# atonderski/future-object-detection

Measured on AMD Instinct MI355X. Metric: frame-sequences/sec fwd+bwd, T=6 900x1600, higher is better.
Workload: dtype bf16; 1 GPU; spatiotemporal ConditionalDETR (ResNet-50, 6 enc + 6 dec layers, 128 queries), T=6 frames 900x1600, batch 2/GPU, num_images K=5 (5 past frames live), random-init weights; step = forward (incl. Hungarian set loss, post-proc, AP bookkeeping) + backward + clip + AdamW; global_batch=2, frames=6, num_images=5, parallelism=dp1

## Files before the change

future-object-detection_amd/csrc/api.cpp:

```cpp
#include <stdarg.h>
#include <stdio.h>
#include <stdlib.h>
#include <string.h>

#include <mutex>

#include "../../include/fod.h"
#include "knobs.h"

static thread_local char g_err[512] = "";

void fod_set_error(const char* fmt, ...) {
  va_list ap;
  va_start(ap, fmt);
  vsnprintf(g_err, sizeof(g_err), fmt, ap);
  va_end(ap);
}

extern "C" size_t fod_last_error(char* buf, size_t cap) {
  const size_t n = strlen(g_err);
  if (buf && cap) {
    const size_t c = n < cap - 1 ? n : cap - 1;
    memcpy(buf, g_err, c);
    buf[c] = 0;
  }
  return n;
}

extern "C" int fod_abi_version(void) { return FOD_ABI_VERSION; }

extern "C" size_t fod_workspace_bytes(int kind) {
  switch (kind) {
    case FOD_WS_NT_SPLIT: return (size_t)FOD_NT_SPLIT_WS_FLOATS * sizeof(float);
    case FOD_WS_NT_SPLIT_TICKETS: return (size_t)FOD_NT_SPLIT_TICKETS * sizeof(unsigned);
    case FOD_WS_TN_PARTIALS: return FOD_TN_WS_BYTES;
    case FOD_WS_ATTN_SPLIT_PER_TILE: return (size_t)FOD_ATTN_SPLIT_WS_FLOATS_PER_TILE * sizeof(float);
    case FOD_WS_DET: return FOD_DET_WS_BYTES;
    case FOD_WS_TN_MULTI_DET: return FOD_TN_MULTI_DET_WS_BYTES;
    default: return 0;
  }
}

namespace {
struct KnobName {
  const char* name;
  int Knobs::*i;
  double Knobs::*d;
};
const KnobName KNOB_NAMES[] = {
    {"FOD_NT_SMALL", &Knobs::nt_small, nullptr},
    {"FOD_NT_NARROW", &Knobs::nt_narrow, nullptr},
    {"FOD_NT_SPLITK", &Knobs::nt_splitk, nullptr},
    {"FOD_NT_BIG", &Knobs::nt_big, nullptr},
    {"FOD_NT_BIG256", &Knobs::nt_big256, nullptr},
    {"FOD_NT_BIG_ILV", &Knobs::nt_big_ilv, nullptr},
    {"FOD_NT_BIG256_MINK", &Knobs::nt_big256_mink, nullptr},
    {"FOD_NT_BIG_MINK", &Knobs::nt_big_mink, nullptr},
    {"FOD_NT_BIG_MINN", &Knobs::nt_big_minn, nullptr},
    {"FOD_TN_SMALL", &Knobs::tn_small, nullptr},
    {"FOD_TN_BIG", &Knobs::tn_big, nullptr},
    {"FOD_TN_BIG_DENSE", &Knobs::tn_big_dense, nullptr},
    {"FOD_TN_BIG256", &Knobs::tn_big256, nullptr},
    {"FOD_TN_BIG_MIN", nullptr, &Knobs::tn_big_min},
    {"FOD_TN_BIG_SPLITS", &Knobs::tn_big_splits, nullptr},
    {"FOD_TN_WS", &Knobs::tn_ws, nullptr},
    {"FOD_TN_XCD", &Knobs::tn_xcd, nullptr},
    {"FOD_TN_ROWS", &Knobs::tn_rows, nullptr},
    {"FOD_ATTN_LDS", &Knobs::attn_lds, nullptr},
    {"FOD_ATTN_PF", &Knobs::attn_pf, nullptr},
    {"FOD_FP8_STAGE", &Knobs::fp8_stage, nullptr},
    {"FOD_LN_BWD_GROUPS", &Knobs::ln_bwd_groups, nullptr},
    {"FOD_BNK_VERSION", &Knobs::bnk_version, nullptr},
};

bool knob_parse(const KnobName& k, const char* text, Knobs& t) {
  char* end = nullptr;
  if (k.d) {
    const double v = strtod(text, &end);
    if (end == text || *end) return false;
    t.*k.d = v;
    return true;
  }
  if (Knobs{}.*k.i == Knobs::AUTO && !strcmp(text, "auto")) {
    t.*k.i = Knobs::AUTO;
    return true;
  }
  const long v = strtol(text, &end, 10);
  if (end == text || *end || v < 0 || v > 0x7FFFFFFF) return false;
  t.*k.i = (int)v;
  return true;
}

std::mutex g_knob_mutex;
Knobs& knob_table() {
  static Knobs table = [] {
    Knobs t;
    for (const KnobName& k : KNOB_NAMES)
      if (const char* text = getenv(k.name)) knob_parse(k, text, t);
    return t;
  }();
  return table;
}
const KnobName* knob_find(const char* name) {
  for (const KnobName& k : KNOB_NAMES)
    if (name && !strcmp(name, k.name)) return &k;
  fod_set_error("knob: unknown name %s", name ? name : "(null)");
  return nullptr;
}
}

Knobs fod_knobs() {
  std::lock_guard<std::mutex> lock(g_knob_mutex);
  return knob_table();
}

extern "C" int fod_knob_set(const char* name, const char* value) {
  const KnobName* k = knob_find(name);
  if (!k) return FOD_ERR_ARG;
  std::lock_guard<std::mutex> lock(g_knob_mutex);
  Knobs& t = knob_table();
  if (!value) {
    const Knobs def;
    if (k->d) t.*k->d = def.*k->d;
    else t.*k->i = def.*k->i;
  } else if (!knob_parse(*k, value, t)) {
    fod_set_error("knob: %s cannot be '%s'", name, value);
    return FOD_ERR_ARG;
  }
  return FOD_OK;
}

extern "C" int fod_knob_get(const char* name, char* out, size_t out_bytes) {
  const KnobName* k = knob_find(name);
  if (!k) return FOD_ERR_ARG;
  const Knobs t = fod_knobs();
  char text[32];
  int n;
  if (k->d) n = snprintf(text, sizeof(text), "%.17g", t.*k->d);
  else if (t.*k->i == Knobs::AUTO) n = snprintf(text, sizeof(text), "auto");
  else n = snprintf(text, sizeof(text), "%d", t.*k->i);
  if (out && (size_t)n < out_bytes) memcpy(out, text, (size_t)n + 1);
  else {
    fod_set_error("knob: %zu bytes do not hold the value of %s", out_bytes, name);
    return FOD_ERR_ARG;
  }
  return FOD_OK;
}
```

future-object-detection_amd/csrc/elementwise.hip:

```cpp
#include <stdlib.h>

#include "common.h"
#include "det_reduce.h"
#include "knobs.h"

namespace {

constexpr int MAX_BLOCKS = 2048;

FOD_DEVINL long res_row(long m, int div, int mod) {
  unsigned r = (unsigned)m;
  if (div > 0) r /= (unsigned)div;
  if (mod > 0) r %= (unsigned)mod;
  return (long)r;
}

template <int LPR>
FOD_DEVINL float row_sum(float v) {
#pragma unroll
  for (int o = LPR / 2; o > 0; o >>= 1) v += __shfl_xor(v, o);
  return v;
}
template <typename T, int EPL>
struct SliceAlign {
  static constexpr unsigned B = EPL * sizeof(T);
  static constexpr unsigned VALUE = (B & (~B + 1)) > 16 ? 16 : (B & (~B + 1));
};
template <typename T, int EPL>
FOD_DEVINL void ln_load(float* v, const T* p) {
  T t[EPL];
  __builtin_memcpy(t, __builtin_assume_aligned(p, SliceAlign<T, EPL>::VALUE), EPL * sizeof(T));
#pragma unroll
  for (int i = 0; i < EPL; ++i) v[i] = to_f32(t[i]);
}
template <typename T, int EPL>
FOD_DEVINL void ln_store(T* p, const float* v) {
  T t[EPL];
#pragma unroll
  for (int i = 0; i < EPL; ++i) t[i] = from_f32<T>(v[i]);
  __builtin_memcpy(__builtin_assume_aligned(p, SliceAlign<T, EPL>::VALUE), t, EPL * sizeof(T));
}

template <typename T, int D, int LPR>
__global__ __launch_bounds__(256) void ln_fwd_kernel(const T* __restrict__ x, const T* __restrict__ res,
                                                     int rdiv, int rmod, const float* __restrict__ gamma,
                                                     const float* __restrict__ beta, T* __restrict__ y,
                                                     T* __restrict__ sum_out, float* __restrict__ mean,
                                                     float* __restrict__ rstd, int rows, float eps,
                                                     int group_rows) {
  constexpr int EPL = D / LPR, RPW = 64 / LPR;
  const int lane = threadIdx.x & 63;
  const int sub = lane % LPR, rsel = lane / LPR;
  const int c0 = sub * EPL;
  const long rows_per_block = (long)(blockDim.x >> 6) * RPW;
  float ga[EPL], be[EPL];
  __builtin_memcpy(ga, __builtin_assume_aligned(gamma + c0, SliceAlign<float, EPL>::VALUE), EPL * sizeof(float));
  __builtin_memcpy(be, __builtin_assume_aligned(beta + c0, SliceAlign<float, EPL>::VALUE), EPL * sizeof(float));
  for (long base = (long)blockIdx.x * rows_per_block + (threadIdx.x >> 6) * RPW; base < rows;
       base += (long)gridDim.x * rows_per_block) {
    const long row = base + rsel;
    const bool live = row < rows;
    const long r = live ? row : rows - 1;
    if (group_rows > 0) {
      const long goff = (r / group_rows) * D + c0;
      __builtin_memcpy(ga, __builtin_assume_aligned(gamma + goff, SliceAlign<float, EPL>::VALUE), EPL * sizeof(float));
      __builtin_memcpy(be, __builtin_assume_aligned(beta + goff, SliceAlign<float, EPL>::VALUE), EPL * sizeof(float));
    }
    float v[EPL];
    ln_load<T, EPL>(v, x + r * D + c0);
    if (res) {
      float t[EPL];
      ln_load<T, EPL>(t, res + res_row(r, rdiv, rmod) * D + c0);
#pragma unroll
      for (int i = 0; i < EPL; ++i) v[i] += t[i];
    }
    if (sum_out) {
      T st[EPL];
#pragma unroll
      for (int i = 0; i < EPL; ++i) {
        st[i] = from_f32<T>(v[i]);
        v[i] = to_f32(st[i]);
      }
      if (live) __builtin_memcpy(__builtin_assume_aligned(sum_out + r * D + c0, SliceAlign<T, EPL>::VALUE), st, EPL * sizeof(T));
    }
    float s = 0.f;
#pragma unroll
    for (int i = 0; i < EPL; ++i) s += v[i];
    const float mu = row_sum<LPR>(s) * (1.f / D);
    float q = 0.f;
#pragma unroll
    for (int i = 0; i < EPL; ++i) q += (v[i] - mu) * (v[i] - mu);
    const float rs = rsqrtf(row_sum<LPR>(q) * (1.f / D) + eps);
    float o[EPL];
#pragma unroll
    for (int i = 0; i < EPL; ++i) o[i] = (v[i] - mu) * rs * ga[i] + be[i];
    if (live) {
      ln_store<T, EPL>(y + r * D + c0, o);
      if (sub == 0) {
        mean[r] = mu;
        rstd[r] = rs;
      }
    }
  }
}

template <typename T, int D, int LPR, bool DET = false>
__global__ __launch_bounds__(256) void ln_bwd_kernel(const T* __restrict__ dy, const T* __restrict__ xs,
                                                     const float* __restrict__ mean,
                                                     const float* __restrict__ rstd,
                                                     const float* __restrict__ gamma, T* __restrict__ dx,
                                                     float* __restrict__ dgamma, float* __restrict__ dbeta,
                                                     int rows, int group_rows) {
  constexpr int EPL = D / LPR, RPW = 64 / LPR;
  __shared__ float sg[4][D];
  __shared__ float sb[4][D];
  const int lane = threadIdx.x & 63, w = threadIdx.x >> 6;
  const int sub = lane % LPR, rsel = lane / LPR;
  const int c0 = sub * EPL;
  float ga[EPL];
  __builtin_memcpy(ga, __builtin_assume_aligned(gamma + c0, SliceAlign<float, EPL>::VALUE), EPL * sizeof(float));
  float ag[EPL], ab[EPL];
#pragma unroll
  for (int i = 0; i < EPL; ++i) ag[i] = ab[i] = 0.f;
  if (group_rows > 0) {
    const long row = (long)blockIdx.x * 4 + w;
    if (row >= rows) return;
    const long goff = (row / group_rows) * D + c0;
    __builtin_memcpy(ga, __builtin_assume_aligned(gamma + goff, SliceAlign<float, EPL>::VALUE), EPL * sizeof(float));
    const float mu = mean[row], rs = rstd[row];
    float d[EPL], g[EPL], xh[EPL];
    ln_load<T, EPL>(d, dy + row * D + c0);
    ln_load<T, EPL>(xh, xs + row * D + c0);
    float s1 = 0.f, s2 = 0.f;
#pragma unroll
    for (int i = 0; i < EPL; ++i) {
      xh[i] = (xh[i] - mu) * rs;
      g[i] = d[i] * ga[i];
      s1 += g[i];
      s2 += g[i] * xh[i];
    }
    s1 = row_sum<LPR>(s1) * (1.f / D);
    s2 = row_sum<LPR>(s2) * (1.f / D);
    float o[EPL];
#pragma unroll
    for (int i = 0; i < EPL; ++i) o[i] = rs * (g[i] - s1 - xh[i] * s2);
    ln_store<T, EPL>(dx + row * D + c0, o);
#pragma unroll
    for (int i = 0; i < EPL; ++i) {
      if (DET) {
        dgamma[row * (2 * D) + c0 + i] = d[i] * xh[i];
        dgamma[row * (2 * D) + D + c0 + i] = d[i];
      } else {
        atomicAdd(dgamma + goff + i, d[i] * xh[i]);
        atomicAdd(dbeta + goff + i, d[i]);
      }
    }
    return;
  }
  for (long base = (long)blockIdx.x * (4 * RPW) + w * RPW; base < rows; base += (long)gridDim.x * (4 * RPW)) {
    const long row = base + rsel;
    const bool live = row < rows;
    const long r = live ? row : rows - 1;
    const float mu = mean[r], rs = rstd[r];
    float d[EPL], g[EPL], xh[EPL];
    ln_load<T, EPL>(d, dy + r * D + c0);
    ln_load<T, EPL>(xh, xs + r * D + c0);
    float s1 = 0.f, s2 = 0.f;
#pragma unroll
    for (int i = 0; i < EPL; ++i) {
      if (!live) d[i] = 0.f;
      xh[i] = (xh[i] - mu) * rs;
      g[i] = d[i] * ga[i];
      s1 += g[i];
      s2 += g[i] * xh[i];
      ag[i] += d[i] * xh[i];
      ab[i] += d[i];
    }
    s1 = row_sum<LPR>(s1) * (1.f / D);
    s2 = row_sum<LPR>(s2) * (1.f / D);
    float o[EPL];
#pragma unroll
    for (int i = 0; i < EPL; ++i) o[i] = rs * (g[i] - s1 - xh[i] * s2);
    if (live) ln_store<T, EPL>(dx + r * D + c0, o);
  }
#pragma unroll
  for (int i = 0; i < EPL; ++i) {
#pragma unroll
    for (int o = LPR; o < 64; o <<= 1) {
      ag[i] += __shfl_xor(ag[i], o);
      ab[i] += __shfl_xor(ab[i], o);
    }
  }
  if (rsel == 0) {
#pragma unroll
    for (int i = 0; i < EPL; ++i) {
      sg[w][c0 + i] = ag[i];
      sb[w][c0 + i] = ab[i];
    }
  }
  __syncthreads();
  for (int c = threadIdx.x; c < D; c += 256) {
    if (DET) {
      dgamma[(long)blockIdx.x * (2 * D) + c] = sg[0][c] + sg[1][c] + sg[2][c] + sg[3][c];
      dgamma[(long)blockIdx.x * (2 * D) + D + c] = sb[0][c] + sb[1][c] + sb[2][c] + sb[3][c];
    } else {
      atomicAdd(dgamma + c, sg[0][c] + sg[1][c] + sg[2][c] + sg[3][c]);
      atomicAdd(dbeta + c, sb[0][c] + sb[1][c] + sb[2][c] + sb[3][c]);
    }
  }
}

template <typename T>
__global__ void eltwise_vec_kernel(int op, T* __restrict__ out, const T* __restrict__ a, const T* __restrict__ b,
                                   const T* __restrict__ c, unsigned nchunks, int cpr, int bdiv, int bmod,
                                   float alpha) {
  constexpr int VEC = Elem<T>::VEC;
  for (unsigned i = blockIdx.x * blockDim.x + threadIdx.x; i < nchunks; i += gridDim.x * blockDim.x) {
    const unsigned m = i / (unsigned)cpr;
    const unsigned col = (i - m * (unsigned)cpr) * VEC;
    T ta[VEC], tb[VEC], tc[VEC], to[VEC];
    __builtin_memcpy(ta, __builtin_assume_aligned(a + (long)i * VEC, 16), 16);
    if (b) __builtin_memcpy(tb, __builtin_assume_aligned(b + res_row(m, bdiv, bmod) * ((long)cpr * VEC) + col, 16), 16);
    if (op == FOD_EW_ADD3) __builtin_memcpy(tc, __builtin_assume_aligned(c + (long)i * VEC, 16), 16);
#pragma unroll
    for (int e = 0; e < VEC; ++e) {
      const float av = to_f32(ta[e]);
      const float bv = b ? to_f32(tb[e]) : 0.f;
      float r;
      switch (op) {
        case FOD_EW_ADD: r = av + bv; break;
        case FOD_EW_MUL: r = av * bv; break;
        case FOD_EW_RELU_MASK: r = bv > 0.f ? av : 0.f; break;
        case FOD_EW_SCALE: r = alpha * av; break;
        case FOD_EW_ADD3: r = av + bv + to_f32(tc[e]); break;
        case FOD_EW_COPY_B: r = bv; break;
        default: r = fmaxf(av, 0.f); break;
      }
      to[e] = from_f32<T>(r);
    }
    __builtin_memcpy(__builtin_assume_aligned(out + (long)i * VEC, 16), to, 16);
  }
}

template <typename T>
__global__ void eltwise_kernel(int op, T* __restrict__ out, const T* __restrict__ a, const T* __restrict__ b,
                               const T* __restrict__ c, long n, int cols, int bdiv, int bmod, float alpha) {
  for (long i = (long)blockIdx.x * blockDim.x + threadIdx.x; i < n; i += (long)gridDim.x * blockDim.x) {
    const long m = i / cols;
    const int col = (int)(i - m * cols);
    const float av = to_f32(a[i]);
    float bv = 0.f;
    if (b) bv = to_f32(b[res_row(m, bdiv, bmod) * cols + col]);
    float r;
    switch (op) {
      case FOD_EW_ADD: r = av + bv; break;
      case FOD_EW_MUL: r = av * bv; break;
      case FOD_EW_RELU_MASK: r = bv > 0.f ? av : 0.f; break;
      case FOD_EW_SCALE: r = alpha * av; break;
      case FOD_EW_ADD3: r = av + bv + to_f32(c[i]); break;
      case FOD_EW_COPY_B: r = bv; break;
      default: r = fmaxf(av, 0.f); break;
    }
    out[i] = from_f32<T>(r);
  }
}

template <typename TS, typename TD>
__global__ void permute3_kernel(const TS* __restrict__ src, TD* __restrict__ dst, int d0, int d1, int d2, long s0,
                                long s1, long s2, int valid2, const float* __restrict__ scale, int axis) {
  const long n = (long)d0 * d1 * d2;
  for (long i = (long)blockIdx.x * blockDim.x + threadIdx.x; i < n; i += (long)gridDim.x * blockDim.x) {
    const int i2 = (int)(i % d2);
    const long t = i / d2;
    const int i1 = (int)(t % d1);
    const int i0 = (int)(t / d1);
    float v = 0.f;
    if (i2 < valid2) {
      v = to_f32(src[i0 * s0 + i1 * s1 + i2 * s2]);
      if (scale) v *= scale[axis == 0 ? i0 : (axis == 1 ? i1 : i2)];
    }
    dst[i] = from_f32<TD>(v);
  }
}

constexpr int MP_CHUNK = 8192;

__host__ __device__ inline int mp_fast_dim(const fod_permute_job& j) {
  if (j.s2 == 1 || j.d2 == 1) return 2;
  if (j.s1 == 1 && j.d1 > 1) return 1;
  if (j.s0 == 1 && j.d0 > 1) return 0;
  return -1;
}

template <typename TS, typename TD>
FOD_DEVINL void multi_permute_body(const fod_permute_job& j, long chunk, float* tile) {
  const TS* __restrict__ src = reinterpret_cast<const TS*>(j.src);
  TD* __restrict__ dst = reinterpret_cast<TD*>(j.dst);
  const unsigned d0 = j.d0, d1 = j.d1, d2 = j.d2;
  const int fast = mp_fast_dim(j);
  const int tid = threadIdx.x;
  if (fast == 0 || fast == 1) {
    const unsigned df = fast == 1 ? d1 : d0, dg = fast == 1 ? d0 : d1;
    const long sg = fast == 1 ? j.s0 : j.s1;
    const unsigned tiles2 = (d2 + 255) / 256, tilesf = (df + 31) / 32;
    const unsigned c = (unsigned)chunk;
    const unsigned t2 = c % tiles2, rest = c / tiles2;
    const unsigned tf = rest % tilesf, ig = rest / tilesf;
    if (ig >= dg) return;
    const unsigned f0 = tf * 32, c0 = t2 * 256;
    if (df <= 16) {
      TS v[16];
#pragma unroll
      for (unsigned k = 0; k < 16; ++k) {
        const unsigned e = tid + 256 * k;
        const unsigned cc = e / df, ifx = e - cc * df;
        const unsigned i2 = c0 + cc;
        const unsigned i1 = fast == 1 ? ifx : ig;
        const bool ok = k < df && i2 < d2 && i1 < (unsigned)j.valid1 && i2 < (unsigned)j.valid2;
        v[k] = src[ok ? (long)ig * sg + ifx + (long)i2 * j.s2 : 0];
        if (!ok) v[k] = from_f32<TS>(0.f);
      }
#pragma unroll
      for (unsigned k = 0; k < 16; ++k) {
        const unsigned e = tid + 256 * k;
        const unsigned cc = e / df, ifx = e - cc * df;
        if (k < df) tile[ifx * 257 + cc] = to_f32(v[k]);
      }
    } else {
    const unsigned lf = tid & 31, lc = tid >> 5;
    TS v[32];
#pragma unroll
    for (unsigned k = 0; k < 32; ++k) {
      const unsigned cc = lc + 8 * k;
      const unsigned i2 = c0 + cc, ifx = f0 + lf;
      const unsigned i1 = fast == 1 ? ifx : ig;
      const bool ok = ifx < df && i2 < d2 && i1 < (unsigned)j.valid1 && i2 < (unsigned)j.valid2;
      v[k] = src[ok ? (long)ig * sg + ifx + (long)i2 * j.s2 : 0];
      if (!ok) v[k] = from_f32<TS>(0.f);
    }
#pragma unroll
    for (unsigned k = 0; k < 32; ++k) tile[lf * 257 + lc + 8 * k] = to_f32(v[k]);
    }
    __syncthreads();
    if (sizeof(TD) == 2 && c0 + 256 <= d2 && ((j.t0 | j.t1) & 7) == 0 && (reinterpret_cast<uintptr_t>(dst) & 15) == 0) {
      const unsigned l8 = (tid & 31) * 8, rr = tid >> 5;
      for (unsigned r = rr; r < 32; r += 8) {
        const unsigned ifx = f0 + r;
        if (ifx >= df) continue;
        const unsigned i0 = fast == 1 ? ig : ifx, i1 = fast == 1 ? ifx : ig;
        const unsigned i2 = c0 + l8;
        TD o[8];
#pragma unroll
        for (int e = 0; e < 8; ++e) {
          float v = tile[r * 257 + l8 + e];
          if (j.scale) v *= j.scale[j.scale_axis == 0 ? i0 : (j.scale_axis == 1 ? i1 : i2 + e)];
          o[e] = from_f32<TD>(v);
        }
        __builtin_memcpy(__builtin_assume_aligned(dst + (long)i0 * j.t0 + (long)i1 * j.t1 + i2, 16), o, 16);
      }
      return;
// ... 373 lines not shown
}

template <typename T>
__global__ void box_finish_bwd_kernel(const float* __restrict__ dboxes, const float* __restrict__ boxes,
                                      const float* __restrict__ ref, T* __restrict__ dt, float* __restrict__ dref,
                                      int levels, int R, int ref_rows) {
  const int n = ref_rows * 4;
  for (int i = blockIdx.x * blockDim.x + threadIdx.x; i < n; i += gridDim.x * blockDim.x) {
    const int k = i & 3, rr = i >> 2;
    float acc = 0.f;
    for (int l = 0; l < levels; ++l)
      for (int r = rr; r < R; r += ref_rows) {
        const long idx = ((long)l * R + r) * 4 + k;
        const float b = boxes[idx];
        const float g = dboxes[idx] * b * (1.f - b);
        dt[idx] = from_f32<T>(g);
        acc += g;
      }
    if (k < 2) dref[rr * 2 + k] += acc * inv_sigmoid_grad(ref[rr * 2 + k]);
  }
}

inline int grid_for(long n, int per_block = 256) {
  long b = (n + per_block - 1) / per_block;
  if (b > MAX_BLOCKS) b = MAX_BLOCKS;
  if (b < 1) b = 1;
  return (int)b;
}

}

#define FOD_DISPATCH_T(dtype, NAME, ...)                         \
  if ((dtype) == FOD_BF16) { using T = __bf16; __VA_ARGS__; }    \
  else if ((dtype) == FOD_F32) { using T = float; __VA_ARGS__; } \
  else { fod_set_error(NAME ": bad dtype %d", (dtype)); return FOD_ERR_ARG; }

extern "C" int fod_layernorm_fwd(int dtype, const void* x, const void* residual, int res_row_div, int res_row_mod,
                                 const float* gamma, const float* beta, void* y, void* sum_out, float* mean,
                                 float* rstd, int rows, int D, float eps, int group_rows, hipStream_t stream) {
  FOD_REQUIRE(x && gamma && beta && y && mean && rstd && rows > 0, "layernorm_fwd: bad args");
  FOD_REQUIRE(group_rows >= 0 && (group_rows == 0 || rows % group_rows == 0), "layernorm_fwd: %d rows in groups of %d", rows, group_rows);
  FOD_REQUIRE(D % 64 == 0 && D >= 64 && D <= 512, "layernorm_fwd: D=%d must be a multiple of 64, <= 512", D);
  FOD_REQUIRE(((uintptr_t)x % 16) == 0 && ((uintptr_t)y % 16) == 0 && ((uintptr_t)residual % 16) == 0 &&
              ((uintptr_t)sum_out % 16) == 0 && ((uintptr_t)gamma % 16) == 0 && ((uintptr_t)beta % 16) == 0,
              "layernorm_fwd: operands must be 16-byte aligned");
#define LN_FWD(DD)                                                                                            \
  do {                                                                                                        \
    constexpr int LPR = (DD % 128 == 0) ? 16 : 8;                                                             \
    if (rows < 8192) {                                                                                        \
      hipLaunchKernelGGL((ln_fwd_kernel<T, DD, 64>), dim3(grid_for(rows, 4)), dim3(256), 0, stream,           \
                         (const T*)x, (const T*)residual, res_row_div, res_row_mod, gamma, beta, (T*)y,       \
                         (T*)sum_out, mean, rstd, rows, eps, group_rows);                                     \
    } else {                                                                                                  \
      hipLaunchKernelGGL((ln_fwd_kernel<T, DD, LPR>), dim3(grid_for(rows, 4 * (64 / LPR))), dim3(256), 0,     \
                         stream, (const T*)x, (const T*)residual, res_row_div, res_row_mod, gamma, beta,      \
                         (T*)y, (T*)sum_out, mean, rstd, rows, eps, group_rows);                              \
    }                                                                                                         \
  } while (0)
  FOD_DISPATCH_T(dtype, "layernorm_fwd", switch (D / 64) {
    case 1: LN_FWD(64); break; case 2: LN_FWD(128); break; case 3: LN_FWD(192); break; case 4: LN_FWD(256); break;
    case 5: LN_FWD(320); break; case 6: LN_FWD(384); break; case 7: LN_FWD(448); break; default: LN_FWD(512); break; })
#undef LN_FWD
  FOD_LAUNCH_CHECK();
  return FOD_OK;
}

static int ln_bwd_groups() {
  const int n = fod_knobs().ln_bwd_groups;
  return n >= 1 && n <= 16 ? n : 4;
}

extern "C" int fod_layernorm_bwd(int dtype, const void* dy, const void* xsum, const float* mean, const float* rstd,
                                 const float* gamma, void* dx, float* dgamma, float* dbeta, int rows, int D,
                                 int group_rows, hipStream_t stream) {
  FOD_REQUIRE(dy && xsum && mean && rstd && gamma && dx && dgamma && dbeta && rows > 0, "layernorm_bwd: bad args");
  FOD_REQUIRE(group_rows >= 0 && (group_rows == 0 || (rows % group_rows == 0 && rows <= 4096)),
              "layernorm_bwd: %d rows in groups of %d (grouped form: at most 4096 rows)", rows, group_rows);
  FOD_REQUIRE(D % 64 == 0 && D >= 64 && D <= 512, "layernorm_bwd: D=%d must be a multiple of 64, <= 512", D);
  FOD_REQUIRE(((uintptr_t)dy % 16) == 0 && ((uintptr_t)xsum % 16) == 0 && ((uintptr_t)dx % 16) == 0 &&
              ((uintptr_t)gamma % 16) == 0, "layernorm_bwd: operands must be 16-byte aligned");
#define LN_BWD(DD)                                                                                            \
  do {                                                                                                        \
    constexpr int LPR = (DD % 128 == 0) ? 16 : 8;                                                             \
    if (rows < 8192) {                                                                                        \
      int grid = grid_for(rows, 16);                                                                          \
      if (grid > 512) grid = 512;                                                                             \
      if (group_rows > 0) grid = (rows + 3) / 4;                              \
      hipLaunchKernelGGL((ln_bwd_kernel<T, DD, 64>), dim3(grid), dim3(256), 0, stream, (const T*)dy,          \
                         (const T*)xsum, mean, rstd, gamma, (T*)dx, dgamma, dbeta, rows, group_rows);         \
    } else {                                                                                                  \
      int grid = grid_for(rows, 4 * (64 / LPR) * ln_bwd_groups());      \
      if (grid > 512) grid = 512;                                                                             \
      hipLaunchKernelGGL((ln_bwd_kernel<T, DD, LPR>), dim3(grid), dim3(256), 0, stream, (const T*)dy,         \
                         (const T*)xsum, mean, rstd, gamma, (T*)dx, dgamma, dbeta, rows, 0);                  \
    }                                                                                                         \
  } while (0)
  FOD_DISPATCH_T(dtype, "layernorm_bwd", switch (D / 64) {
    case 1: LN_BWD(64); break; case 2: LN_BWD(128); break; case 3: LN_BWD(192); break; case 4: LN_BWD(256); break;
    case 5: LN_BWD(320); break; case 6: LN_BWD(384); break; case 7: LN_BWD(448); break; default: LN_BWD(512); break; })
#undef LN_BWD
  FOD_LAUNCH_CHECK();
  return FOD_OK;
}

extern "C" int fod_layernorm_bwd_det(int dtype, const void* dy, const void* xsum, const float* mean, const float* rstd,
                                     const float* gamma, void* dx, float* dgamma, float* dbeta, int rows, int D,
                                     int group_rows, void* ws, size_t ws_bytes, hipStream_t stream) {
  FOD_REQUIRE_SCRATCH("layernorm_bwd_det", ws, ws_bytes, FOD_DET_WS_BYTES);
  FOD_REQUIRE(dy && xsum && mean && rstd && gamma && dx && dgamma && dbeta && rows > 0, "layernorm_bwd_det: bad args");
  FOD_REQUIRE(group_rows >= 0 && (group_rows == 0 || (rows % group_rows == 0 && rows <= 4096)),
              "layernorm_bwd_det: %d rows in groups of %d (grouped form: at most 4096 rows)", rows, group_rows);
  FOD_REQUIRE(D % 64 == 0 && D >= 64 && D <= 512, "layernorm_bwd_det: D=%d must be a multiple of 64, <= 512", D);
  FOD_REQUIRE(((uintptr_t)dy % 16) == 0 && ((uintptr_t)xsum % 16) == 0 && ((uintptr_t)dx % 16) == 0 &&
              ((uintptr_t)gamma % 16) == 0, "layernorm_bwd_det: operands must be 16-byte aligned");
  float* part = reinterpret_cast<float*>(ws);
  int grid = 0;
  const bool few = rows < 8192;
  if (few) {
    grid = grid_for(rows, 16);
    if (grid > 512) grid = 512;
    if (group_rows > 0) grid = (rows + 3) / 4;
  } else {
    FOD_REQUIRE(group_rows == 0, "layernorm_bwd_det: the grouped form takes at most 4096 rows");
  }
#define LN_BWD_DET(DD)                                                                                        \
  do {                                                                                                        \
    constexpr int LPR = (DD % 128 == 0) ? 16 : 8;                                                             \
    if (few) {                                                                                                \
      hipLaunchKernelGGL((ln_bwd_kernel<T, DD, 64, true>), dim3(grid), dim3(256), 0, stream, (const T*)dy,    \
                         (const T*)xsum, mean, rstd, gamma, (T*)dx, part, nullptr, rows, group_rows);         \
    } else {                                                                                                  \
      grid = grid_for(rows, 4 * (64 / LPR) * ln_bwd_groups());                                                \
      if (grid > 512) grid = 512;                                                                             \
      hipLaunchKernelGGL((ln_bwd_kernel<T, DD, LPR, true>), dim3(grid), dim3(256), 0, stream, (const T*)dy,   \
                         (const T*)xsum, mean, rstd, gamma, (T*)dx, part, nullptr, rows, 0);                  \
    }                                                                                                         \
  } while (0)
  FOD_DISPATCH_T(dtype, "layernorm_bwd_det", switch (D / 64) {
    case 1: LN_BWD_DET(64); break; case 2: LN_BWD_DET(128); break; case 3: LN_BWD_DET(192); break;
    case 4: LN_BWD_DET(256); break; case 5: LN_BWD_DET(320); break; case 6: LN_BWD_DET(384); break;
    case 7: LN_BWD_DET(448); break; default: LN_BWD_DET(512); break; })
#undef LN_BWD_DET
  FOD_LAUNCH_CHECK();
  const int nparts = group_rows > 0 ? group_rows : grid;
  const int groups = group_rows > 0 ? rows / group_rows : 1;
  foddet::ReduceParams r{};
  r.part = part; r.part_stride = 2L * D; r.part_batch = (long)nparts * 2 * D; r.part_total = r.part_batch; r.nparts = nparts;
  r.out0 = dgamma; r.n0 = D; r.cols0 = D; r.ld0 = D; r.out0_batch = D;
  r.out1 = dbeta; r.n1 = D; r.out1_batch = D;
  r.accumulate = 1;
  return det_reduce_launch(r, groups, stream);
}

struct ColsumJob {
  const void* g;
  void* out;
};
constexpr int COLSUM_MAX_JOBS = 16;
struct ColsumJobs {
  ColsumJob j[COLSUM_MAX_JOBS];
};
__global__ __launch_bounds__(256) void colsum_groups_multi_kernel(const ColsumJobs jobs, int group_rows, int N) {
  __shared__ __attribute__((aligned(16))) float red[4][256];
  const int tx = threadIdx.x & 63, rl = threadIdx.x >> 6;
  const int grp = blockIdx.x;
  const __bf16* G = reinterpret_cast<const __bf16*>(jobs.j[blockIdx.y].g) + (long)grp * group_rows * N;
  const bool in = 4 * tx < N;
  float a0 = 0.f, a1 = 0.f, a2 = 0.f, a3 = 0.f;
  if (in) {
    int m = rl;
    for (; m + 28 < group_rows; m += 32) {
      bf16x4_t v[8];
#pragma unroll
      for (int k = 0; k < 8; ++k) v[k] = *reinterpret_cast<const bf16x4_t*>(G + (long)(m + 4 * k) * N + 4 * tx);
#pragma unroll
      for (int k = 0; k < 8; ++k) {
        a0 += (float)v[k][0]; a1 += (float)v[k][1]; a2 += (float)v[k][2]; a3 += (float)v[k][3];
      }
    }
    for (; m < group_rows; m += 4) {
      const bf16x4_t v = *reinterpret_cast<const bf16x4_t*>(G + (long)m * N + 4 * tx);
      a0 += (float)v[0]; a1 += (float)v[1]; a2 += (float)v[2]; a3 += (float)v[3];
    }
  }
  *reinterpret_cast<f32x4*>(&red[rl][4 * tx]) = f32x4{a0, a1, a2, a3};
  __syncthreads();
  if (rl == 0 && in) {
    f32x4 t = *reinterpret_cast<const f32x4*>(&red[0][4 * tx]);
    t += *reinterpret_cast<const f32x4*>(&red[1][4 * tx]);
    t += *reinterpret_cast<const f32x4*>(&red[2][4 * tx]);
    t += *reinterpret_cast<const f32x4*>(&red[3][4 * tx]);
    __bf16* o = reinterpret_cast<__bf16*>(jobs.j[blockIdx.y].out) + (long)grp * N + 4 * tx;
    *reinterpret_cast<bf16x4_t*>(o) = bf16x4_t{(__bf16)t[0], (__bf16)t[1], (__bf16)t[2], (__bf16)t[3]};
  }
}

extern "C" int fod_colsum_groups_multi(int dtype, int njobs, const void* const* ptrs, int groups, int group_rows, int N,
                                       hipStream_t stream) {
  FOD_REQUIRE(dtype == FOD_BF16, "colsum_groups_multi: bf16 only (dtype %d)", dtype);
  FOD_REQUIRE(ptrs && njobs > 0 && njobs <= COLSUM_MAX_JOBS, "colsum_groups_multi: 1 .. %d jobs (%d)", COLSUM_MAX_JOBS, njobs);
  FOD_REQUIRE(groups > 0 && groups <= 65535 && group_rows > 0 && N > 0 && N <= 256 && N % 4 == 0,
              "colsum_groups_multi: %d groups of %d rows, N = %d (N <= 256, a multiple of 4)", groups, group_rows, N);
  ColsumJobs jobs{};
  for (int i = 0; i < njobs; ++i) {
    jobs.j[i].g = ptrs[2 * i];
    jobs.j[i].out = const_cast<void*>(ptrs[2 * i + 1]);
    FOD_REQUIRE(jobs.j[i].g && jobs.j[i].out && ((uintptr_t)jobs.j[i].g % 8) == 0 && ((uintptr_t)jobs.j[i].out % 8) == 0,
                "colsum_groups_multi: job %d: null or misaligned operand", i);
  }
  hipLaunchKernelGGL(colsum_groups_multi_kernel, dim3(groups, njobs), dim3(256), 0, stream, jobs, group_rows, N);
  FOD_LAUNCH_CHECK();
  return FOD_OK;
}

extern "C" int fod_eltwise(int op, int dtype, void* out, const void* a, const void* b, const void* c, long rows,
                           int cols, int b_row_div, int b_row_mod, float alpha, hipStream_t stream) {
  FOD_REQUIRE(out && a && rows > 0 && cols > 0 && rows < (1L << 31), "eltwise: bad args");
  FOD_REQUIRE(op >= FOD_EW_ADD && op <= FOD_EW_COPY_B, "eltwise: bad op %d", op);
  FOD_REQUIRE(b || op == FOD_EW_SCALE || op == FOD_EW_RELU, "eltwise: op %d needs b", op);
  FOD_REQUIRE(c || op != FOD_EW_ADD3, "eltwise: ADD3 needs c");
  const long n = rows * cols;
  const int vec = dtype == FOD_BF16 ? 8 : 4;
  auto al = [](const void* q) { return ((uintptr_t)q % 16) == 0; };
  if (cols % vec == 0 && n / vec < (1L << 32) - 1 && al(out) && al(a) && (!b || al(b)) && (!c || al(c))) {
    FOD_DISPATCH_T(dtype, "eltwise",
                   hipLaunchKernelGGL((eltwise_vec_kernel<T>), dim3(grid_for(n / vec)), dim3(256), 0, stream, op,
                                      (T*)out, (const T*)a, (const T*)b, (const T*)c, (unsigned)(n / vec), cols / vec,
                                      b_row_div, b_row_mod, alpha))
    FOD_LAUNCH_CHECK();
    return FOD_OK;
  }
  FOD_DISPATCH_T(dtype, "eltwise",
                 hipLaunchKernelGGL((eltwise_kernel<T>), dim3(grid_for(n)), dim3(256), 0, stream, op, (T*)out,
                                    (const T*)a, (const T*)b, (const T*)c, n, cols, b_row_div, b_row_mod, alpha))
  FOD_LAUNCH_CHECK();
  return FOD_OK;
}

extern "C" int fod_dropout(int dtype, void* out, const void* a, long n, unsigned long long seed,
                           const unsigned long long* seed_dev, float p, hipStream_t stream) {
  const int vec = dtype == FOD_BF16 ? 8 : 4;
  FOD_REQUIRE(out && a && n > 0 && n % vec == 0 && n < (1L << 32), "dropout: bad size %ld", n);
  FOD_REQUIRE(p >= 0.f && p < 1.f, "dropout: p=%f out of [0, 1)", p);
  FOD_REQUIRE(((uintptr_t)out % 16) == 0 && ((uintptr_t)a % 16) == 0, "dropout: operands must be 16-byte aligned");
  const unsigned threshold = (unsigned)((double)p * 4294967296.0);
  const float inv_keep = 1.f / (1.f - p);
  FOD_DISPATCH_T(dtype, "dropout",
                 hipLaunchKernelGGL((dropout_kernel<T>), dim3(grid_for(n / vec)), dim3(256), 0, stream, (T*)out,
                                    (const T*)a, (unsigned)(n / vec), seed, seed_dev, threshold, inv_keep))
  FOD_LAUNCH_CHECK();
  return FOD_OK;
}

extern "C" int fod_permute3_cast(int src_dtype, int dst_dtype, const void* src, void* dst, int d0, int d1, int d2,
                                 long s0, long s1, long s2, int valid2, const float* scale, int scale_axis,
                                 hipStream_t stream) {
  FOD_REQUIRE(src && dst && d0 > 0 && d1 > 0 && d2 > 0, "permute3: bad args");
  const long n = (long)d0 * d1 * d2;
  const dim3 grid(grid_for(n)), block(256);
#define P3(TS, TD) \
  hipLaunchKernelGGL((permute3_kernel<TS, TD>), grid, block, 0, stream, (const TS*)src, (TD*)dst, d0, d1, d2, s0, s1, s2, valid2, scale, scale_axis)
  if (src_dtype == FOD_F32 && dst_dtype == FOD_F32) P3(float, float);
  else if (src_dtype == FOD_F32 && dst_dtype == FOD_BF16) P3(float, __bf16);
  else if (src_dtype == FOD_BF16 && dst_dtype == FOD_F32) P3(__bf16, float);
  else if (src_dtype == FOD_BF16 && dst_dtype == FOD_BF16) P3(__bf16, __bf16);
  else { fod_set_error("permute3: bad dtypes %d %d", src_dtype, dst_dtype); return FOD_ERR_ARG; }
#undef P3
  FOD_LAUNCH_CHECK();
  return FOD_OK;
}

extern "C" int fod_multi_permute3(const fod_permute_job* jobs, const int* blk_job, const int* blk_chunk, int nblocks,
                                  hipStream_t stream) {
  FOD_REQUIRE(jobs && blk_job && blk_chunk && nblocks > 0, "multi_permute3: bad args");
  hipLaunchKernelGGL(multi_permute3_kernel, dim3(nblocks), dim3(256), 0, stream, jobs, blk_job, blk_chunk);
  FOD_LAUNCH_CHECK();
  return FOD_OK;
}

extern "C" int fod_multi_permute_chunk(void) { return MP_CHUNK; }

extern "C" int fod_multi_permute_tiles(int d0, int d1, int d2, long s0, long s1, long s2) {
  fod_permute_job j{};
  j.d0 = d0; j.d1 = d1; j.d2 = d2; j.s0 = s0; j.s1 = s1; j.s2 = s2;
  const int fast = mp_fast_dim(j);
  if (fast == 0 || fast == 1) {
    const long df = fast == 1 ? d1 : d0, dg = fast == 1 ? d0 : d1;
    return (int)(((d2 + 255) / 256) * ((df + 31) / 32) * dg);
  }
  const long n = (long)d0 * d1 * d2;
  if (n >= (1L << 31)) return -1;
  return (int)((n + MP_CHUNK - 1) / MP_CHUNK);
}

extern "C" int fod_nchw_to_nhwc(int dtype, const float* src, void* dst, int F, int C, int H, int W, int Cp,
                                int inner, long stride_outer, long stride_inner, hipStream_t stream) {
  FOD_REQUIRE(src && dst && F > 0 && C > 0 && Cp >= C && inner > 0 && F % inner == 0, "nchw_to_nhwc: bad args");
  const long n = (long)F * H * W;
  const long hw = (long)H * W;
  if (dtype == FOD_BF16 && Cp == 8 && hw % 4 == 0 && stride_outer % 4 == 0 && stride_inner % 4 == 0 &&
      (reinterpret_cast<uintptr_t>(src) & 15) == 0 && (reinterpret_cast<uintptr_t>(dst) & 15) == 0 && F <= 65535) {
    const int bx = (int)std::min<long>((hw / 4 + 255) / 256, 512);
    hipLaunchKernelGGL(nchw_to_nhwc8_kernel, dim3(bx, F), dim3(256), 0, stream, src, (__bf16*)dst, C, hw, inner,
                       stride_outer, stride_inner);
    FOD_LAUNCH_CHECK();
    return FOD_OK;
// ... 132 lines not shown
```

future-object-detection_amd/csrc/knobs.h:

```cpp
#pragma once

struct Knobs {
  static constexpr int AUTO = -1;
  int nt_small = 1;
  int nt_narrow = AUTO;
  int nt_splitk = AUTO;
  int nt_big = 1;
  int nt_big256 = 1;
  int nt_big_ilv = AUTO;
  int nt_big256_mink = 128;
  int nt_big_mink = 1536;
  int nt_big_minn = 256;
  int tn_small = 1;
  int tn_big = 1;
  int tn_big_dense = 0;
  int tn_big256 = 0;
  double tn_big_min = 2.0e9;
  int tn_big_splits = 0;
  int tn_ws = 1;
  int tn_xcd = 1;
  int tn_rows = 0;
  int attn_lds = 8;
  int attn_pf = 1;
  int fp8_stage = 1;
  int ln_bwd_groups = 4;
  int bnk_version = 4;
};

Knobs fod_knobs();
```

future-object-detection_amd/future_od/models/transformer.py:

```python
import math
from typing import List, Optional

import torch
from torch import Tensor, nn

from future_od.native import functional as Fn
from future_od.native import ops
from future_od.switches import SW


def _reset_parameters(parameters):
    for p in parameters:
        if p.dim() > 1:
            nn.init.xavier_uniform_(p)


def _lin(x, m: nn.Linear, relu=False, out_f32=False):
    return Fn.linear(x, m.weight, m.bias, relu=relu, out_f32=out_f32)


class _Proj:
    __slots__ = ("a", "lin", "a_relu")

    def __init__(self, a, lin, a_relu=False):
# ... 198 lines not shown
    for qc, qs, side, layer, image in blocks:
        kc, ks, _v = side.slots(layer, image)
        jobs.append((qc.detach().contiguous(), qs.detach().contiguous(), kc.detach(), ks.detach()))
    D = blocks[0][0].shape[-1]
    return ops.attn_maps(jobs, 1.0 / math.sqrt(2 * D // nhead), query_idx)


@torch.no_grad()
def _head_mean_weights(qc, kc, qs, ks, H):
    B, M, D = qc.shape
    N = kc.shape[1]
    hd = D // H
    q = torch.cat([qc.float().view(B, M, H, hd), qs.float().view(B, M, H, hd)], 3).transpose(1, 2)
    k = torch.cat([kc.float().view(B, N, H, hd), ks.float().view(B, N, H, hd)], 3).transpose(1, 2)
    w = torch.softmax(q @ k.transpose(-1, -2) / math.sqrt(2 * hd), dim=-1)
    return w.mean(1)


class TransformerDecoderLayer(nn.Module):

    def __init__(self, D, Nhead, Dff=2048, dropout=0.1, num_images=1, use_slotstates=False, use_egodeep=False):
        super().__init__()
        self.self_attend = SlotToSlotAttention(D, Nhead, dropout)
        self.norm_sa = nn.LayerNorm(D)
        self.image_attend = nn.ModuleList([SlotToImageAttention(D, Nhead, dropout) for _ in range(num_images)])
        self.norm_ia = nn.ModuleList([nn.LayerNorm(D) for _ in range(num_images)])
        if use_slotstates:
            self.slotstates_attend = SlotToSlotAttention(D, Nhead, dropout)
            self.norm_ssa = nn.LayerNorm(D)
        else:
            self.slotstates_attend = None
        if use_egodeep:
            self.egodeep_attend = EgodeepAttention(D, Nhead, droprate=dropout, Dff=None)
            self.norm_eda = nn.LayerNorm(D)
        else:
            self.egodeep_attend = None
        self.feedforward = nn.Sequential(nn.Linear(D, Dff), nn.ReLU(inplace=True), nn.Dropout(dropout),
                                         nn.Linear(Dff, D))
        self.norm_out = nn.LayerNorm(D)
        self.Nhead, self.D = Nhead, D
        self.droprate = dropout

    def forward(self, x, qpos, query_sine, side, layer, is_first=False, pos_proj=None, slotstates=None, egodeep=None):
        t, p = self.training, self.droprate
        o = self.self_attend(x, qpos, pos_proj["sa"] if pos_proj else None)
        if side.K > 0:
            x, qc_pre = _add_norm(x, o, self.norm_sa, p, t, then=self.image_attend[0].query_content)
        else:
            x, qc_pre = _add_norm(x, o, self.norm_sa, p, t), None
        qs_all = Fn.group_linear(query_sine, [self.image_attend[i].query_sine for i in range(side.K)])
        for i in range(side.K):
            o, x = self.image_attend[i](x, qpos, query_sine, side, layer, i, is_first, qs=qs_all[i],
                                        qpos_proj=pos_proj["ca"][i] if (pos_proj and is_first) else None, keep=True,
                                        qc_pre=qc_pre)
            if i + 1 < side.K:
                x, qc_pre = _add_norm(x, o, self.norm_ia[i], p, t, then=self.image_attend[i + 1].query_content)
            else:
                x, qc_pre = _add_norm(x, o, self.norm_ia[i], p, t), None
        if self.slotstates_attend is not None and slotstates is not None:
            o = self.slotstates_attend.forward_cross(x, qpos, slotstates)
            x = _add_norm(x, o, self.norm_ssa, p, t)
        if self.egodeep_attend is not None and egodeep is not None and egodeep.dim() == 2 and self.egodeep_attend.per_token_masks():
            egodeep = egodeep.unsqueeze(1)
        if self.egodeep_attend is not None and egodeep is not None and egodeep.dim() == 3:
            e = Fn.dropout(self.egodeep_attend.forward_keys(x, qpos, egodeep), p, t)
            x = Fn.layer_norm(x, self.norm_eda.weight, self.norm_eda.bias, residual=e)
        elif self.egodeep_attend is not None and egodeep is not None:
            e = Fn.dropout(self.egodeep_attend.forward_single_key(egodeep), p, t)
            x = Fn.layer_norm(x, self.norm_eda.weight, self.norm_eda.bias, residual=e, res_row_div=x.shape[1])
            if torch.is_grad_enabled():
                x = Fn.ZeroGradAnchor.apply(x, *self.egodeep_attend.dead_parameters())
        fuse = _fused_tail(self.feedforward[3], p, t)
        x, h = Fn.linear_keep(x, self.feedforward[0].weight, self.feedforward[0].bias, relu=True, grad_masked=fuse)
        h = Fn.dropout(h, p, t)
        return _add_norm(x, _Proj(h, self.feedforward[3], a_relu=fuse), self.norm_out, p, t)


class TransformerDecoder(nn.Module):

    def __init__(self, layers, norm=None, return_intermediate=False, D=256):
        super().__init__()
        self.layers = layers
        for module in self.layers[1:]:
            for att in module.image_attend:
                att.query_pos.weight = None
                att.query_pos.bias = None
        self.norm = norm
        self.return_intermediate = return_intermediate
        self.D = D
        self.query_scale = MLP(D, D, D, 2)
        self.ref_point_head = MLP(D, D, 2, 2)
        _reset_parameters(self.parameters())

    def forward(self, x, qpos, mems, mem_poss, first_layer_special=True, slotstates=None, egodeep=None):
        B, M, D = x.shape
        ref, sine0 = Fn.RefPointSineFn.apply(self.ref_point_head(qpos), D)
        K = len(mems)
        big = [Fn.wide_linear(mems[j], [m for layer in self.layers
                                        for m in (layer.image_attend[j].value, layer.image_attend[j].key_content)])
               for j in range(K)]
        ks_all = Fn.wide_linear(mem_poss[0], [layer.image_attend[j].key_pos for layer in self.layers for j in range(K)])
        side = Fn.MemorySide(big, ks_all, len(self.layers), K, D)
        pos_lin = [m for layer in self.layers for m in (layer.self_attend.query_pos, layer.self_attend.key_pos)]
        if first_layer_special:
            pos_lin += [self.layers[0].image_attend[j].query_pos for j in range(K)]
        pos_all = Fn.group_linear(qpos, pos_lin)
        inter = []
        sine_acc, first_scaled = Fn.TableGradAcc(), True
        for lid, layer in enumerate(self.layers):
            special = lid == 0 and first_layer_special
            pos_proj = {"sa": (pos_all[2 * lid], pos_all[2 * lid + 1]),
                        "ca": pos_all[2 * len(self.layers):] if special else None}
            if special:
                q_sine = sine0
            elif Fn.mlp2_mul_fits(x, self.query_scale, sine0):
                q_sine = Fn.mlp2_mul(x.view(B * M, D), self.query_scale, sine0, acc=sine_acc,
                                     hands_on=first_scaled).view(B, M, D)
                first_scaled = False
            else:
                q_sine = Fn.mul(self.query_scale(x).view(B * M, D), sine0, b_row_mod=M).view(B, M, D)
            x = layer(x, qpos, q_sine, side, lid, is_first=special, pos_proj=pos_proj, slotstates=slotstates,
                      egodeep=egodeep)
            if self.return_intermediate:
                inter.append(x)
        if not self.return_intermediate:
            y = Fn.layer_norm(x, self.norm.weight, self.norm.bias) if self.norm is not None else x
            return y.unsqueeze(0), ref
        return Fn.layer_norm(torch.stack(inter), self.norm.weight, self.norm.bias), ref


class PackedMHA(nn.Module):

    def __init__(self, D):
        super().__init__()
        self.in_proj_weight = nn.Parameter(torch.empty(3 * D, D))
        self.in_proj_bias = nn.Parameter(torch.zeros(3 * D))
        self.out_proj = nn.Linear(D, D)
        nn.init.xavier_uniform_(self.in_proj_weight)
        nn.init.constant_(self.out_proj.bias, 0.0)


class EncoderAttention(nn.Module):

    def __init__(self, Dsrc, num_heads, Dff, droprate=0.1):
        super().__init__()
        self.attn = PackedMHA(Dsrc)
        self.norm1 = nn.LayerNorm(Dsrc)
        self.mlp = nn.Sequential(nn.Linear(Dsrc, Dff), nn.ReLU(inplace=True), nn.Dropout(droprate),
                                 nn.Linear(Dff, Dsrc), nn.Dropout(droprate))
        self.norm2 = nn.LayerNorm(Dsrc)
        self.D, self.H = Dsrc, num_heads
        self.droprate = droprate

    def forward(self, src, pos, other=None, attn_mask=None, key_padding_mask=None):
        _no_masks(attn_mask, key_padding_mask)
        D = self.D
        N = pos.shape[-2]
        add_pos = (lambda t: Fn.add(t, pos, b_row_mod=N)) if pos.dim() == 2 else (lambda t: Fn.add(t, pos))
        fused = Fn.in_proj_self(src, pos, self.attn.in_proj_weight, self.attn.in_proj_bias) if other is None else None
        if fused is not None:
            src, q, k, v = fused
        elif other is None:
            q, k, v = Fn.in_proj(add_pos(src), src, self.attn.in_proj_weight, self.attn.in_proj_bias)
        else:
            q, k, v = Fn.in_proj_cross(add_pos(src), add_pos(other), other, self.attn.in_proj_weight,
                                       self.attn.in_proj_bias)
        a = Fn.attention(q, k, v, 1.0 / math.sqrt(D // self.H), drop_p=self.droprate, training=self.training)
        t, p = self.training, self.droprate
        src = _add_norm(src, _Proj(a, self.attn.out_proj), self.norm1, p, t)
        fuse = _fused_tail(self.mlp[3], p, t)
        src, h = Fn.linear_keep(src, self.mlp[0].weight, self.mlp[0].bias, relu=True, grad_masked=fuse)
        h = Fn.dropout(h, p, t)
        return _add_norm(src, _Proj(h, self.mlp[3], a_relu=fuse), self.norm2, p, t)


class TransformerEncoderLayer(nn.Module):

    def __init__(self, D, Nhead, Dff=2048, droprate=0.1, num_previmages=0, use_prevout=False, use_egodeep=False):
        super().__init__()
        self.self_attn = EncoderAttention(D, Nhead, Dff, droprate=droprate)
        self.prevout_attn = EncoderAttention(D, Nhead, Dff, droprate=droprate) if use_prevout else None
        self.previmage_attn = nn.ModuleList(
            [EncoderAttention(D, Nhead, Dff, droprate=droprate) for _ in range(num_previmages)])
        if use_egodeep:
            self.egodeep_attend = EgodeepAttention(D, Nhead, droprate=droprate, Dff=Dff)
            self.norm_eda = nn.LayerNorm(D)
        else:
            self.egodeep_attend = None

    def forward(self, x, pos, egodeep: Optional[Tensor] = None, prevout: Optional[Tensor] = None, memory=None,
                imu_pre: Optional[Tensor] = None, imu_queue=None):
        x = self.self_attn(x, pos)
        if prevout is not None and self.prevout_attn is not None:
            x = self.prevout_attn(x, pos, other=prevout)
        if memory is not None:
            for prev, attn in zip(memory, self.previmage_attn):
                x = attn(x, pos, other=prev)
        if egodeep is not None and self.egodeep_attend is not None and egodeep.dim() == 2 and self.egodeep_attend.per_token_masks():
            egodeep = egodeep.unsqueeze(1)
        if egodeep is not None and self.egodeep_attend is not None and egodeep.dim() == 3:
            e = self.egodeep_attend.forward_keys(x, pos, egodeep)
            e = Fn.dropout(e, self.egodeep_attend.droprate, self.training)
            x = Fn.layer_norm(x, self.norm_eda.weight, self.norm_eda.bias, residual=e)
        elif egodeep is not None and self.egodeep_attend is not None:
            N = x.shape[1]
            e = imu_pre if imu_pre is not None else self.egodeep_attend.forward_single_key(egodeep)
            e = Fn.dropout(e, self.egodeep_attend.droprate, self.training)
            if imu_queue is not None and e is imu_pre:
                x = Fn.layer_norm(x, self.norm_eda.weight, self.norm_eda.bias, residual=e, res_row_div=N,
                                  res_queue=imu_queue[0], res_slot=imu_queue[1])
            else:
                x = Fn.layer_norm(x, self.norm_eda.weight, self.norm_eda.bias, residual=e, res_row_div=N)
            if torch.is_grad_enabled():
                x = Fn.ZeroGradAnchor.apply(x, *self.egodeep_attend.dead_parameters())
        return x


class TransformerEncoder(nn.Module):
    def __init__(self, layers):
        super().__init__()
        self.layers = layers
        _reset_parameters(self.parameters())

    def forward(self, x, pos, egodeep: Optional[Tensor] = None, prevout: Optional[Tensor] = None, memory=None):
        pre = None
        blocks = [getattr(layer, "egodeep_attend", None) for layer in self.layers]
        if (egodeep is not None and egodeep.dim() == 2 and all(b is not None for b in blocks)
                and not any(b.training and b.droprate > 0.0 for b in blocks) and Fn.imu_branch_fits(egodeep, blocks)):
            queue = Fn.ResGradQueue(len(blocks)) if (SW.FOD_RES_GRAD_QUEUE and torch.is_grad_enabled()) else None
            pre = Fn.imu_branch(egodeep, blocks, queue=queue)
        for i, layer in enumerate(self.layers):
            if pre is not None:
                x = layer(x, pos, egodeep, prevout, memory, imu_pre=pre[i],
                          imu_queue=None if queue is None else (queue, i))
            else:
                x = layer(x, pos, egodeep, prevout, memory)
        return x
```

future-object-detection_amd/future_od/native/functional.py:

```python
import torch
from torch.autograd import Function

from . import lib as L
from . import ops
from .arena import ARENA, _ZeroArena, zeros_f32
from .prepared import (CAT, PREP, STACK, _Job, _Prepared, _VEC, _pad_to, _wkey, prep_conv, prep_linear,
                       prep_stem)
from .wgrad import WGRADS, _WgradQueue
from ..switches import SW

GRAD_SYNC = None


set_deterministic = ops.set_deterministic
is_deterministic = ops.is_deterministic


def set_grad_sync(reducer):
    global GRAD_SYNC
    GRAD_SYNC = reducer


class BackboneCut:

    def __init__(self):
        self.pairs = []

    def cut(self, feat):
        leaf = feat.detach().requires_grad_(True)
        self.pairs.append((feat, leaf))
        return leaf

    def finish(self):
        pairs, self.pairs = self.pairs, []
        if pairs:
            torch.autograd.backward([f for f, _ in pairs], [l.grad for _, l in pairs])


BACKBONE_CUT = None


def cast(t, dtype, pad_cols=None):
    cols = t.shape[-1]
    rows = t.numel() // cols
    t = t.contiguous()
    pc = cols if pad_cols is None else pad_cols
    return ops.permute3_cast(t, dtype, (1, rows, pc), (0, cols, 1), valid2=cols).view(*t.shape[:-1], pc)


def _grad_rows(dy, cols, dtype):
    g = dy.contiguous().view(-1, cols)
    return g if g.dtype == dtype else cast(g, dtype)


def _param_grads(weight, bias, g, x, need_w, need_b, shared):
    want_db = bias is not None and need_b
    if shared and need_w and WGRADS.chain(weight, want_db, g, x):
        return None, None
    db = zeros_f32((g.shape[-1],), x.device) if want_db else None
    dw = None
    if need_w:
        dw = zeros_f32((g.shape[-1], x.shape[-1]), x.device)
        WGRADS.tn(WGRADS.site((weight, bias)), g, x, dw, db, owner=weight if shared else None)
    elif want_db:
        ops.colsum_acc(g, db)
    return dw, db


class LinearFn(Function):

    @staticmethod
    def forward(ctx, x, weight, bias, relu, out_f32):
        dtype = x.dtype
        w = prep_linear(weight, dtype, False)
        N = weight.shape[0]
        y = ops.gemm_nt(x, w[:N] if w.shape[0] != N else w, shift=bias, relu=relu, out_f32=out_f32)
        y = y.view(*x.shape[:-1], N)
        ctx.relu, ctx.out_f32 = relu, out_f32
        ctx.weight, ctx.bias = weight, bias
        ctx.has_bias = bias is not None
        ctx.save_for_backward(x, y if relu else None)
        return y

    @staticmethod
    def backward(ctx, dy):
        x, y = ctx.saved_tensors
        weight = ctx.weight
        dtype = x.dtype
        N, K = weight.shape
        v = _VEC[dtype]
        Np = _pad_to(N, v)
        dy = dy.contiguous()
        if dy.dtype != dtype or Np != N:
            g = cast(dy.view(-1, N), dtype, pad_cols=Np)
        else:
            g = dy.view(-1, N)
        if ctx.relu:
            assert Np == N
            g = ops.eltwise(L.EW_RELU_MASK, g, y.view(-1, N))
        dx = None
        if ctx.needs_input_grad[0]:
            dx = ops.gemm_nt(g, prep_linear(weight, dtype, True)).view(x.shape)
        dw, db = _param_grads(weight, ctx.bias, g, x.view(-1, K), ctx.needs_input_grad[1], ctx.needs_input_grad[2], True)
        if Np != N:
            dw, db = (None if dw is None else dw[:N]), (None if db is None else db[:N])
        return dx, dw, db, None, None


def linear(x, weight, bias=None, relu=False, out_f32=False):
    return LinearFn.apply(x.contiguous(), weight, bias, relu, out_f32)


class LinearKeepFn(Function):

    @staticmethod
    def forward(ctx, x, weight, bias, relu, grad_masked=False, precomputed=None):
        dtype = x.dtype
        N = weight.shape[0]
        if precomputed is not None:
            y = precomputed.view(*x.shape[:-1], N)
        else:
            w = prep_linear(weight, dtype, False)
            y = ops.gemm_nt(x, w[:N] if w.shape[0] != N else w, shift=bias, relu=relu).view(*x.shape[:-1], N)
        ctx.relu, ctx.weight, ctx.bias, ctx.has_bias = relu, weight, bias, bias is not None
        ctx.mask_here = relu and not grad_masked
        ctx.save_for_backward(x, y if ctx.mask_here else None)
        return x.view_as(x), y

    @staticmethod
    def backward(ctx, dkeep, dy):
        x, y = ctx.saved_tensors
        weight = ctx.weight
        dtype = x.dtype
        N, K = weight.shape
        assert N % _VEC[dtype] == 0
        g = _grad_rows(dy, N, dtype)
        if ctx.mask_here:
            g = ops.eltwise(L.EW_RELU_MASK, g, y.view(-1, N))
        dx = None
        if ctx.needs_input_grad[0]:
            res = None if dkeep is None else _grad_rows(dkeep, K, dtype)
            dx = ops.gemm_nt(g, prep_linear(weight, dtype, True), residual=res).view(x.shape)
        dw, db = _param_grads(weight, ctx.bias, g, x.view(-1, K), ctx.needs_input_grad[1], ctx.needs_input_grad[2], False)
        return dx, dw, db, None, None, None


def linear_keep(x, weight, bias=None, relu=False, grad_masked=False, precomputed=None):
    if weight.shape[0] % _VEC[x.dtype] != 0 or not SW.FOD_LINEAR_KEEP:
        assert precomputed is None
        return x, linear(x, weight, bias, relu=relu)
    return LinearKeepFn.apply(x.contiguous(), weight, bias, relu, grad_masked, precomputed)


class AddFn(Function):

    @staticmethod
    def forward(ctx, a, b, b_row_div, b_row_mod):
        ctx.cfg = (b_row_div, b_row_mod, b.shape, a.shape)
        return ops.eltwise(L.EW_ADD, a, b, b_row_div=b_row_div, b_row_mod=b_row_mod)

    @staticmethod
    def backward(ctx, g):
        div, mod, bshape, ashape = ctx.cfg
        g = g.contiguous()
        db = None
        if ctx.needs_input_grad[1]:
            cols = ashape[-1]
            rows = g.numel() // cols
            if not div and not mod:
                db = g.view(bshape)
            elif mod and not div:
                db = _sum_periodic(g.view(rows, cols), mod).view(bshape)
            else:
                assert not mod
                out = zeros_f32((rows // div, cols), g.device)
                ops.colsum_acc(g.view(rows, cols), out, group_rows=div)
                db = cast(out, g.dtype).view(bshape)
        return (g.view(ashape) if ctx.needs_input_grad[0] else None), db, None, None


def add(a, b, b_row_div=0, b_row_mod=0):
    return AddFn.apply(a.contiguous(), b.contiguous(), b_row_div, b_row_mod)


class MulFn(Function):

    @staticmethod
    def forward(ctx, a, b, b_row_mod):
        ctx.save_for_backward(a, b)
        ctx.mod = b_row_mod
        return ops.eltwise(L.EW_MUL, a, b, b_row_mod=b_row_mod)

    @staticmethod
    def backward(ctx, g):
        a, b = ctx.saved_tensors
        g = g.contiguous()
        da = ops.eltwise(L.EW_MUL, g, b, b_row_mod=ctx.mod)
        db = ops.eltwise(L.EW_MUL, g, a)
        if ctx.mod:
            db = _sum_periodic(db, ctx.mod).view(b.shape)
        return da, db, None


class TableGradAcc:

    def __init__(self):
        self.buf = None

    def get(self, shape, device):
        if self.buf is None:
            self.buf = zeros_f32(shape, device)
        return self.buf

    def take(self):
        buf, self.buf = self.buf, None
        return buf


class Mlp2MulFn(Function):

    @staticmethod
    def forward(ctx, x, table, w1, b1, w2, b2, acc, hands_on):
        D = x.shape[-1]
        x2 = x.view(-1, D)
        out, h, q = ops.mlp2_mul_fwd(x2, prep_linear(w1, x.dtype, False), b1, prep_linear(w2, x.dtype, False), b2, table)
        ctx.save_for_backward(x2, h, q, table)
        ctx.params, ctx.acc, ctx.hands_on, ctx.x_shape = (w1, b1, w2, b2), acc, hands_on, x.shape
        return out.view(x.shape)

    @staticmethod
    def backward(ctx, g):
        x2, h, q, table = ctx.saved_tensors
        w1, b1, w2, b2 = ctx.params
        D = x2.shape[-1]
        g = _grad_rows(g, D, x2.dtype)
        acc = ctx.acc if ctx.acc is not None else TableGradAcc()
        buf = acc.get(tuple(table.shape), x2.device)
        ds, dh, dx = ops.mlp2_mul_bwd(g, table, q, h, prep_linear(w2, x2.dtype, True), prep_linear(w1, x2.dtype, True), buf)
        dw2, db2 = _param_grads(w2, b2, ds, h, ctx.needs_input_grad[4], ctx.needs_input_grad[5], True)
        dw1, db1 = _param_grads(w1, b1, dh, x2, ctx.needs_input_grad[2], ctx.needs_input_grad[3], True)
        dtable = None
        if ctx.needs_input_grad[1] and (ctx.acc is None or ctx.hands_on):
            dtable = cast(acc.take(), table.dtype).view(table.shape)
        return (dx.view(ctx.x_shape) if ctx.needs_input_grad[0] else None), dtable, dw1, db1, dw2, db2, None, None


def mlp2_mul_fits(x, mlp, table):
    if not SW.FOD_FUSED_MLP2 or x.dtype != torch.bfloat16 or getattr(mlp, "num_layers", 0) != 2:
        return False
    l0, l1 = mlp.layers
    D = x.shape[-1]
    return (D == 256 and tuple(l0.weight.shape) == (D, D) and tuple(l1.weight.shape) == (D, D) and l0.bias is not None
            and l1.bias is not None and table.dtype == x.dtype and table.dim() == 2 and table.shape[1] == D
            and (x.numel() // D) % table.shape[0] == 0)


def mlp2_mul(x, mlp, table, acc=None, hands_on=True):
    l0, l1 = mlp.layers
    return Mlp2MulFn.apply(x.contiguous(), table.contiguous(), l0.weight, l0.bias, l1.weight, l1.bias, acc, hands_on)


def _sum_periodic(g, mod):
    parts = g.view(-1, mod, g.shape[-1])
# ... 260 lines not shown
DROP_SEEDS = _DropSeeds()


def manual_seed(seed):
    torch.manual_seed(seed)
    DROP_SEEDS.count = 0
    if ops.DROP_BASE is not None:
        ops.DROP_BASE.zero_()


class DropoutFn(Function):
    @staticmethod
    def forward(ctx, x, p, seed):
        ctx.p, ctx.seed = p, seed
        return ops.dropout(x, p, seed)

    @staticmethod
    def backward(ctx, g):
        return ops.dropout(g.contiguous(), ctx.p, ctx.seed), None, None


def dropout(x, p, training):
    if not training or p <= 0.0:
        return x
    return DropoutFn.apply(x.contiguous(), float(p), DROP_SEEDS.next())


def _fp8_takes(q1, k1, drop_p):
    mode = SW.FOD_ATTN_FP8
    if mode == "off" or q1.dtype != torch.bfloat16 or drop_p > 0.0:
        return False
    few_queries = q1.shape[1] <= 512 and k1.shape[1] >= 128
    return mode == "all" or not few_queries


class AttentionFn(Function):
    @staticmethod
    def forward(ctx, q1, k1, v, q2, k2, scale, drop_p=0.0, drop_seed=0):
        ctx.drop = (drop_p, drop_seed)
        ctx.scale = scale
        ctx.two = q2 is not None
        ctx.fp8 = _fp8_takes(q1, k1, drop_p)
        if ctx.fp8:
            need_bwd = any(t is not None and t.requires_grad for t in (q1, k1, v, q2, k2))
            o, lse2, deq = ops.attn_fwd_fp8(q1, k1, v, scale, q2, k2, want_backward=need_bwd)
            if need_bwd:
                ctx.save_for_backward(deq[0], deq[1], deq[2], deq[3], deq[4], o, lse2)
            return o
        o, lse2 = ops.attn_fwd(q1, k1, v, scale, q2, k2, drop_p=drop_p, drop_seed=drop_seed)
        ctx.save_for_backward(q1, k1, v, q2, k2, o, lse2)
        return o

    @staticmethod
    def backward(ctx, do):
        q1, k1, v, q2, k2, o, lse2 = ctx.saved_tensors
        slots = {}
        qk = _column_siblings(q1, k1)
        if qk is not None:
            D = q1.shape[-1]
            dqk = torch.empty_strided(qk.shape, qk.stride(), dtype=qk.dtype, device=qk.device)
            slots = dict(dq1_out=dqk[..., :D], dk1_out=dqk[..., D:])
        elif q1.shape == k1.shape == v.shape and q1.is_contiguous() and k1.is_contiguous() and v.is_contiguous():
            buf = torch.empty((3,) + tuple(q1.shape), dtype=q1.dtype, device=q1.device)
            slots = dict(dq1_out=buf[0], dk1_out=buf[1], dv_out=buf[2])
        if ctx.fp8:
            dq1, dk1, dq2, dk2, dv = ops.attn_bwd(q1, k1, v, o, do.contiguous(), lse2, 1.0 / ops.LOG2E, q2, k2,
                                                  dq_scale=ctx.scale * ops.LOG2E, **slots)
            return dq1, dk1, dv, dq2, dk2, None, None, None
        dq1, dk1, dq2, dk2, dv = ops.attn_bwd(q1, k1, v, o, do.contiguous(), lse2, ctx.scale, q2, k2,
                                              drop_p=ctx.drop[0], drop_seed=ctx.drop[1], **slots)
        return dq1, dk1, dv, dq2, dk2, None, None, None


def _strided_ok(t):
    v = _VEC[t.dtype]
    return (t.dim() == 3 and t.stride(-1) == 1 and t.stride(0) % v == 0 and t.stride(1) % v == 0
            and t.data_ptr() % 16 == 0)


def attention(q1, k1, v, scale, q2=None, k2=None, drop_p=0.0, training=False):
    c = lambda t: None if t is None else (t if _strided_ok(t) else t.contiguous())
    drop = (float(drop_p), DROP_SEEDS.next()) if training and drop_p > 0.0 else ()
    return AttentionFn.apply(c(q1), c(k1), c(v), c(q2), c(k2), scale, *drop)


def _column_siblings(a, b):
    D = a.shape[-1]
    if (b is None or a.shape != b.shape or a.stride() != b.stride() or a.stride(-1) != 1 or a.stride(-2) != 2 * D
            or a.untyped_storage().data_ptr() != b.untyped_storage().data_ptr()
            or b.storage_offset() != a.storage_offset() + D):
        return None
    outer = 2 * D
    for n, st in zip(reversed(a.shape[:-1]), reversed(a.stride()[:-1])):
        if st != outer:
            return None
        outer *= n
    return torch.as_strided(a, tuple(a.shape[:-1]) + (2 * D,), a.stride())


class InProjFn(Function):

    @staticmethod
    def forward(ctx, xp, src, w, b):
        return _in_proj_forward(ctx, xp, src, w, b)

    @staticmethod
    def backward(ctx, dq, dk, dv):
        return _in_proj_backward(ctx, dq, dk, dv, ctx.needs_input_grad[0], ctx.needs_input_grad[1])


def _in_proj_forward(ctx, xp, src, w, b):
    D = w.shape[1]
    dtype = xp.dtype
    wqk, wv = prep_linear(w[:2 * D], dtype, False), prep_linear(w[2 * D:], dtype, False)
    qk = ops.gemm_nt(xp, wqk, shift=b[:2 * D]).view(*xp.shape[:-1], 2 * D)
    v = ops.gemm_nt(src, wv, shift=b[2 * D:]).view(src.shape)
    ctx.save_for_backward(xp, src)
    ctx.w, ctx.b = w, b
    return qk[..., :D], qk[..., D:], v


def _in_proj_backward(ctx, dq, dk, dv, need_xp, need_src, chained=False, dkeep=None):
    xp, src = ctx.saved_tensors
    w, b = ctx.w, ctx.b
    D = w.shape[1]
    dtype = xp.dtype
    rows = xp.numel() // D
    dqk = _column_siblings(dq, dk)
    if dqk is None:
        dqk = torch.cat([dq, dk], dim=-1)
    dqk = dqk.reshape(rows, 2 * D)
    dv = dv.contiguous().view(rows, D)
    dxp = dsrc = None
    if need_xp:
        res = None if dkeep is None else _grad_rows(dkeep, D, dtype)
        dxp = ops.gemm_nt(dqk, prep_linear(w[:2 * D], dtype, True), residual=res).view(xp.shape)
    if need_src:
        dsrc = ops.gemm_nt(dv, prep_linear(w[2 * D:], dtype, True), residual=dxp if chained else None).view(src.shape)
    dw = zeros_f32((3 * D, D), xp.device)
    db = zeros_f32((3 * D,), xp.device)
    wq = WGRADS.site((w, b))
    WGRADS.tn(wq, dqk, xp.view(rows, D), dw[:2 * D], db[:2 * D])
    WGRADS.tn(wq, dv, src.view(rows, D), dw[2 * D:], db[2 * D:])
    return dxp, dsrc, dw, db


def in_proj(xp, src, weight, bias):
    return InProjFn.apply(xp.contiguous(), src.contiguous(), weight, bias)


class InProjSelfFn(Function):

    @staticmethod
    def forward(ctx, src, pos, w, b, row_mod):
        xp = ops.eltwise(L.EW_ADD, src, pos, b_row_mod=row_mod)
        return (src.view_as(src),) + _in_proj_forward(ctx, xp, src, w, b)

    @staticmethod
    def backward(ctx, dkeep, dq, dk, dv):
        need = ctx.needs_input_grad[0]
        _, dsrc, dw, db = _in_proj_backward(ctx, dq, dk, dv, need, need, chained=True, dkeep=dkeep)
        return dsrc, None, dw, db, None


def in_proj_self(src, pos, weight, bias):
    if pos.requires_grad or not SW.FOD_LINEAR_KEEP:
        return None
    row_mod = pos.shape[-2] if pos.dim() == 2 else 0
    return InProjSelfFn.apply(src.contiguous(), pos.contiguous(), weight, bias, row_mod)


class InProjCrossFn(Function):

    @staticmethod
    def forward(ctx, xq, xk, xv, w, b):
        D = w.shape[1]
        dtype = xq.dtype
        q = ops.gemm_nt(xq, prep_linear(w[:D], dtype, False), shift=b[:D]).view(xq.shape)
        k = ops.gemm_nt(xk, prep_linear(w[D:2 * D], dtype, False), shift=b[D:2 * D]).view(xk.shape)
        v = ops.gemm_nt(xv, prep_linear(w[2 * D:], dtype, False), shift=b[2 * D:]).view(xv.shape)
        ctx.save_for_backward(xq, xk, xv)
        ctx.w, ctx.b = w, b
        return q, k, v

    @staticmethod
    def backward(ctx, dq, dk, dv):
        xs = ctx.saved_tensors
        w, b = ctx.w, ctx.b
        D = w.shape[1]
        dtype = xs[0].dtype
        dw = zeros_f32((3 * D, D), xs[0].device)
        db = zeros_f32((3 * D,), xs[0].device)
        dxs = []
        wq = WGRADS.site((w, b))
        for i, (x, g) in enumerate(zip(xs, (dq, dk, dv))):
            rows = x.numel() // D
            g = g.contiguous().view(rows, D)
            sl = slice(i * D, (i + 1) * D)
            dxs.append(ops.gemm_nt(g, prep_linear(w[sl], dtype, True)).view(x.shape) if ctx.needs_input_grad[i] else None)
            WGRADS.tn(wq, g, x.view(rows, D), dw[sl], db[sl])
        return dxs[0], dxs[1], dxs[2], dw, db


def in_proj_cross(xq, xk, xv, weight, bias):
    return InProjCrossFn.apply(xq.contiguous(), xk.contiguous(), xv.contiguous(), weight, bias)


class RefPointSineFn(Function):

    @staticmethod
    def forward(ctx, ref_logit, D):
        ref, sine = ops.refpoint_sine_fwd(ref_logit, D)
        ctx.save_for_backward(ref)
        ctx.D, ctx.act_dtype = D, ref_logit.dtype
        return ref, sine

    @staticmethod
    def backward(ctx, dref, dsine):
        (ref,) = ctx.saved_tensors
        if dsine is None:
            dsine = torch.zeros((ref.shape[0], ctx.D), dtype=ctx.act_dtype, device=ref.device)
        return ops.refpoint_sine_bwd(dsine.contiguous(), ref, None if dref is None else dref.contiguous()), None


class BoxFinishFn(Function):

    @staticmethod
    def forward(ctx, t, ref, levels):
        boxes = ops.box_finish_fwd(t, ref, levels)
        ctx.save_for_backward(boxes, ref)
        ctx.act_dtype = t.dtype
        ctx.t_shape = t.shape
        return boxes

    @staticmethod
    def backward(ctx, dboxes):
        boxes, ref = ctx.saved_tensors
        dt_, dref = ops.box_finish_bwd(dboxes.contiguous(), boxes, ref, ctx.act_dtype)
        return dt_.view(ctx.t_shape), dref, None


class ZeroGradAnchor(Function):

    @staticmethod
    def forward(ctx, x, *params):
        ctx.shapes = [(p.shape, p.device) for p in params]
        return x.view_as(x)

    @staticmethod
    def backward(ctx, g):
        return (g,) + tuple(zeros_f32(s, d) for s, d in ctx.shapes)


class CastFn(Function):

    @staticmethod
    def forward(ctx, x, dtype, pad_cols):
        ctx.src_dtype, ctx.cols = x.dtype, x.shape[-1]
        return cast(x, dtype, pad_cols)

    @staticmethod
    def backward(ctx, g):
        g = g.contiguous()
        cols = g.shape[-1]
        rows = g.numel() // cols
        out = ops.permute3_cast(g, ctx.src_dtype, (1, rows, ctx.cols), (0, cols, 1))
        return out.view(*g.shape[:-1], ctx.cols), None, None


def cast_ad(x, dtype, pad_cols=None):
    if x.dtype == dtype and pad_cols in (None, x.shape[-1]):
        return x
    return CastFn.apply(x.contiguous(), dtype, pad_cols)




class WideLinearFn(Function):

    @staticmethod
    def forward(ctx, x, *params):
        P = len(params) // 2
        weights, biases = params[:P], params[P:]
        wcat, bcat, _ = CAT.get(weights, biases, x.dtype)
        y = ops.gemm_nt(x, wcat, shift=bcat).view(*x.shape[:-1], wcat.shape[0])
        ctx.save_for_backward(x)
        ctx.params = params
        return y

    @staticmethod
    def backward(ctx, dy):
        (x,) = ctx.saved_tensors
        P = len(ctx.params) // 2
        weights, biases = ctx.params[:P], ctx.params[P:]
        D_out, D_in = weights[0].shape
        _, _, wcat_t = CAT.get(weights, biases, x.dtype)
        g = dy.contiguous().view(-1, P * D_out)
        dx = None
        if ctx.needs_input_grad[0]:
            dx = ops.gemm_nt(g, wcat_t).view(x.shape)
        dw = zeros_f32((P * D_out, D_in), x.device)
        db = zeros_f32((P * D_out,), x.device)
        WGRADS.tn(WGRADS.site(ctx.params), g, x.view(-1, D_in), dw, db)
        gw = [dw[i * D_out:(i + 1) * D_out] for i in range(P)]
        gb = [db[i * D_out:(i + 1) * D_out] for i in range(P)]
        return (dx,) + tuple(gw) + tuple(gb)


class GroupLinearFn(Function):

    @staticmethod
    def forward(ctx, x, nres, res_mod, *tensors):
        res, params = tensors[:nres], tensors[nres:]
        P = len(params) // 2
        weights, biases = params[:P], params[P:]
        wcat, bcat, _ = CAT.get(weights, biases, x.dtype)
        D = weights[0].shape[0]
        rblock = None
        if nres:
            rblock = _as_segments(res, res[0].numel() // D, D)
            assert rblock is not None, "group_linear(residual=...): the tables must be consecutive blocks (the caller checks)"
        y = ops.group_linear_fwd(x.view(-1, x.shape[-1]), wcat, bcat, P, residual=rblock, res_row_mod=res_mod)
# ... 301 lines not shown
```

future-object-detection_amd/future_od/native/ops.py:

```python
import ctypes as C
import math

import torch

from . import abi, capture
from . import lib as L
from .lib import F32, BF16, AttnShape, ConvGeom, Epilogue
from .. import switches
from ..switches import SW


def call(name, *args, **kw):
    return L.call(name, *args, **kw)

_DT = {torch.float32: F32, torch.bfloat16: BF16}


def dt(t):
    try:
        return _DT[t.dtype]
    except KeyError:
        raise L.FodError(f"unsupported activation dtype {t.dtype}") from None


# ... 848 lines not shown
    if out is None:
        out = torch.empty((B, Q, n, S), dtype=torch.float32, device=q1.device)
    else:
        _chk(out, f"{who}: out", torch.float32)
        if tuple(out.shape) != (B, Q, n, S) or out.device != q1.device:
            raise L.FodError(f"{who}: out {tuple(out.shape)} is not [{B}, {Q}, {n}, {S}] on {q1.device}")
    H = E // 32
    shp = AttnShape(B, H, Tq, S, qb, qt, kb, kt, 0, 0, 0, 0, float(scale), k2b, k2t, 0, 0, 0.0, 0, None, None, None, 0.0)
    parts = 2 if q2 is not None else 1
    call("fod_attn_maps", dt(q1), n, C.addressof(arr), ptr(query_idx), Q, ptr(out), _Addr(shp), stream(),
         work=2.0 * 2 * n * B * H * Q * S * 32 * parts)
    return out


def layernorm_fwd(x, gamma, beta, residual=None, res_row_div=0, res_row_mod=0, want_sum=None, eps=1e-5, group_rows=0):
    _chk(x, "x"); _chk(gamma, "gamma", torch.float32); _chk(beta, "beta", torch.float32)
    D = x.shape[-1]
    rows = x.numel() // D
    if group_rows:
        assert rows % group_rows == 0 and gamma.numel() == (rows // group_rows) * D and beta.numel() == gamma.numel()
    else:
        assert gamma.numel() == D and beta.numel() == D
    if residual is not None:
        _chk(residual, "residual", x.dtype); assert residual.shape[-1] == D
        rr = residual.numel() // D
        need = rows
        if res_row_div:
            need = (rows - 1) // res_row_div + 1
        if res_row_mod:
            need = min(need, res_row_mod)
        assert rr >= need, (x.shape, residual.shape, res_row_div, res_row_mod)
    want_sum = (residual is not None) if want_sum is None else want_sum
    y = torch.empty_like(x)
    s = torch.empty_like(x) if want_sum else None
    mean = torch.empty(rows, dtype=torch.float32, device=x.device)
    rstd = torch.empty(rows, dtype=torch.float32, device=x.device)
    call("fod_layernorm_fwd", dt(x), ptr(x), ptr(residual), res_row_div, res_row_mod, ptr(gamma), ptr(beta),
         ptr(y), ptr(s), ptr(mean), ptr(rstd), rows, D, eps, group_rows, stream())
    return y, (s if want_sum else x), mean, rstd


def linear_add_norm_fwd(a, w, bias, x, gamma, beta, eps=1e-5, then_w=None, then_bias=None):
    _chk(a, "a", torch.bfloat16); _chk(w, "w", torch.bfloat16); _chk(x, "x", torch.bfloat16)
    _chk(gamma, "gamma", torch.float32); _chk(beta, "beta", torch.float32)
    N, K = w.shape
    M = a.numel() // K
    assert a.shape[-1] == K and x.numel() == M * N and gamma.numel() == N and beta.numel() == N, (a.shape, w.shape, x.shape)
    if bias is not None:
        _chk(bias, "bias", torch.float32); assert bias.numel() == N
    y = torch.empty_like(x)
    s = torch.empty_like(x)
    mean = torch.empty(M, dtype=torch.float32, device=x.device)
    rstd = torch.empty(M, dtype=torch.float32, device=x.device)
    out2 = None
    if then_w is not None:
        _chk(then_w, "then_w", torch.bfloat16); assert tuple(then_w.shape) == (N, N)
        if then_bias is not None:
            _chk(then_bias, "then_bias", torch.float32); assert then_bias.numel() == N
        out2 = torch.empty_like(x)
    call("fod_linear_add_norm_fwd", dt(a), ptr(a), K, ptr(w), ptr(bias), ptr(x), ptr(gamma), ptr(beta), ptr(y), ptr(s),
         ptr(mean), ptr(rstd), M, N, K, eps, ptr(then_w), ptr(then_bias), ptr(out2), stream(),
         work=2.0 * M * N * K * (2 if then_w is not None else 1), tag="fod_gemm_nt")
    return (y, s, mean, rstd) if then_w is None else (y, s, mean, rstd, out2)


def linear_add_norm_bwd(dy, xsum, mean, rstd, gamma, w_t, dgamma, dbeta, want_da=True, pre_g=None, pre_w_t=None):
    _chk(xsum, "xsum", torch.bfloat16); _chk(w_t, "w_t", torch.bfloat16)
    K, N = w_t.shape
    M = xsum.numel() // N
    if pre_g is not None:
        _chk(pre_g, "pre_g", torch.bfloat16); _chk(pre_w_t, "pre_w_t", torch.bfloat16)
        assert pre_g.numel() == M * N and tuple(pre_w_t.shape) == (N, N)
    else:
        assert pre_w_t is None and dy is not None
    if dy is not None:
        _chk(dy, "dy", torch.bfloat16); assert dy.numel() == xsum.numel()
    assert mean.numel() == M and rstd.numel() == M and gamma.numel() == N
    _chk(dgamma, "dgamma", torch.float32); _chk(dbeta, "dbeta", torch.float32)
    dsum = torch.empty_like(xsum)
    da = torch.empty((M, K), dtype=xsum.dtype, device=xsum.device) if want_da else None
    call_twin("fod_linear_add_norm_bwd", xsum.device, dt(xsum), ptr(dy), ptr(xsum), ptr(mean), ptr(rstd), ptr(gamma),
              ptr(w_t), ptr(dsum), ptr(da), ptr(dgamma), ptr(dbeta), M, N, K, ptr(pre_g), ptr(pre_w_t),
              work=2.0 * M * N * K * ((1 if want_da else 0) + (1 if pre_g is not None else 0)), tag="fod_gemm_nt")
    return dsum, da


def colsum_groups_multi(jobs, groups, group_rows, N):
    n = len(jobs)
    assert 0 < n <= 16
    arr = (C.c_void_p * (2 * n))()
    for i, (g, out) in enumerate(jobs):
        _chk(g, "g", torch.bfloat16); _chk(out, "out", torch.bfloat16)
        assert g.numel() == groups * group_rows * N and out.numel() == groups * N
        arr[2 * i], arr[2 * i + 1] = g.data_ptr(), out.data_ptr()
    call("fod_colsum_groups_multi", BF16, n, C.addressof(arr), groups, group_rows, N, stream())


def mlp2_mul_fwd(x, w1, b1, w2, b2, table=None):
    _chk(x, "x", torch.bfloat16); _chk(w1, "w1", torch.bfloat16); _chk(w2, "w2", torch.bfloat16)
    D = x.shape[-1]
    M = x.numel() // D
    assert tuple(w1.shape) == (D, D) and tuple(w2.shape) == (D, D), (x.shape, w1.shape, w2.shape)
    for b in (b1, b2):
        if b is not None:
            _chk(b, "bias", torch.float32); assert b.numel() == D
    rows_t = 0
    if table is not None:
        _chk(table, "table", torch.bfloat16); assert table.shape[-1] == D
        rows_t = table.numel() // D
        assert M % rows_t == 0
    h = torch.empty((M, D), dtype=x.dtype, device=x.device)
    q = torch.empty((M, D), dtype=x.dtype, device=x.device) if table is not None else None
    out = torch.empty((M, D), dtype=x.dtype, device=x.device)
    call("fod_mlp2_mul_fwd", dt(x), ptr(x), ptr(w1), ptr(b1), ptr(w2), ptr(b2), ptr(table), rows_t, ptr(h), ptr(q),
         ptr(out), M, D, stream(), work=4.0 * M * D * D, tag="fod_gemm_nt")
    return out, h, q


def mlp2_mul_bwd(dout, table, q, h, w2_t, w1_t, dtable):
    _chk(dout, "dout", torch.bfloat16); _chk(h, "h", torch.bfloat16)
    _chk(w2_t, "w2_t", torch.bfloat16); _chk(w1_t, "w1_t", torch.bfloat16)
    D = dout.shape[-1]
    M = dout.numel() // D
    assert h.numel() == M * D and tuple(w2_t.shape) == (D, D) and tuple(w1_t.shape) == (D, D)
    rows_t = 0
    ds = None
    if table is not None:
        _chk(table, "table", torch.bfloat16); _chk(q, "q", torch.bfloat16); _chk(dtable, "dtable", torch.float32)
        rows_t = table.numel() // D
        assert q.numel() == M * D and dtable.numel() == rows_t * D and M % rows_t == 0
        ds = torch.empty((M, D), dtype=dout.dtype, device=dout.device)
    dh = torch.empty((M, D), dtype=dout.dtype, device=dout.device)
    dx = torch.empty((M, D), dtype=dout.dtype, device=dout.device)
    call_twin("fod_mlp2_mul_bwd", dout.device, dt(dout), ptr(dout), ptr(table), rows_t, ptr(q), ptr(h), ptr(w2_t),
              ptr(w1_t), ptr(ds), ptr(dh), ptr(dx), ptr(dtable), M, D, work=4.0 * M * D * D, tag="fod_gemm_nt")
    return (ds if table is not None else dout), dh, dx


def layernorm_bwd(dy, xsum, mean, rstd, gamma, dgamma, dbeta, group_rows=0):
    _chk(dy, "dy"); _chk(xsum, "xsum", dy.dtype)
    D = dy.shape[-1]
    rows = dy.numel() // D
    assert xsum.numel() == dy.numel() and mean.numel() == rows and rstd.numel() == rows
    groups = rows // group_rows if group_rows else 1
    assert not group_rows or (rows % group_rows == 0 and rows <= 4096)
    for t in (gamma, dgamma, dbeta):
        _chk(t, "gamma/dgamma/dbeta", torch.float32); assert t.numel() == groups * D
    dx = torch.empty_like(dy)
    call_twin("fod_layernorm_bwd", dy.device, dt(dy), ptr(dy), ptr(xsum), ptr(mean), ptr(rstd), ptr(gamma), ptr(dx),
              ptr(dgamma), ptr(dbeta), rows, D, group_rows)
    return dx


def eltwise(op, a, b=None, c=None, b_row_div=0, b_row_mod=0, alpha=1.0, out=None):
    _chk(a, "a")
    cols = a.shape[-1]
    rows = a.numel() // cols
    if b is not None:
        _chk(b, "b", a.dtype); assert b.shape[-1] == cols
        need = rows
        if b_row_div:
            need = (rows - 1) // b_row_div + 1
        if b_row_mod:
            need = min(need, b_row_mod)
        assert b.numel() // cols >= need, (a.shape, b.shape, b_row_div, b_row_mod)
    if c is not None:
        _chk(c, "c", a.dtype); assert c.numel() == a.numel()
    out = torch.empty_like(a) if out is None else out
    call("fod_eltwise", op, dt(a), ptr(out), ptr(a), ptr(b), ptr(c), rows, cols, b_row_div, b_row_mod,
         float(alpha), stream())
    return out


def add(a, b, **kw):
    return eltwise(L.EW_ADD, a, b, **kw)


DROP_BASE = None


def dropout(a, p, seed):
    _chk(a, "a")
    out = torch.empty_like(a)
    call("fod_dropout", dt(a), ptr(out), ptr(a), a.numel(), seed & 0xFFFFFFFFFFFFFFFF, ptr(DROP_BASE), float(p), stream())
    return out


def posenc_table(h, w, c, dtype, device, temperature=10000.0):
    out = torch.empty((h * w, c), dtype=dtype, device=device)
    call("fod_posenc_table", _DT[dtype], ptr(out), h, w, c, temperature, stream())
    return out


def posenc_temporal(b, l, c, dtype, device, offsets=None, extra=0.0, temperature=10000.0):
    out = torch.empty((b, l, c), dtype=dtype, device=device)
    if offsets is not None:
        _chk(offsets, "offsets", torch.float32); assert offsets.shape == (b, l)
    call("fod_posenc_temporal", _DT[dtype], ptr(out), ptr(offsets), b, l, c, extra, temperature, stream())
    return out


def refpoint_sine_fwd(ref_logit, D):
    _chk(ref_logit, "ref_logit")
    R = ref_logit.numel() // 2
    ref = torch.empty((R, 2), dtype=torch.float32, device=ref_logit.device)
    sine = torch.empty((R, D), dtype=ref_logit.dtype, device=ref_logit.device)
    call("fod_refpoint_sine_fwd", dt(ref_logit), ptr(ref_logit), ptr(ref), ptr(sine), R, D, stream())
    return ref, sine


def refpoint_sine_bwd(dsine, ref, dref_extra):
    _chk(dsine, "dsine"); _chk(ref, "ref", torch.float32)
    R, D = dsine.shape
    assert ref.shape == (R, 2)
    if dref_extra is not None:
        _chk(dref_extra, "dref_extra", torch.float32); assert dref_extra.shape == (R, 2)
    out = torch.empty((R, 2), dtype=dsine.dtype, device=dsine.device)
    call("fod_refpoint_sine_bwd", dt(dsine), ptr(dsine), ptr(ref), ptr(dref_extra), ptr(out), R, D, stream())
    return out


def box_finish_fwd(t, ref, levels):
    _chk(t, "t"); _chk(ref, "ref", torch.float32)
    ref_rows = ref.shape[0]
    assert t.numel() % (levels * 4) == 0
    R = t.numel() // (levels * 4)
    assert R % ref_rows == 0 and ref.shape == (ref_rows, 2)
    boxes = torch.empty((levels, R, 4), dtype=torch.float32, device=t.device)
    call("fod_box_finish_fwd", dt(t), ptr(t), ptr(ref), ptr(boxes), levels, R, ref_rows, stream())
    return boxes


def box_finish_bwd(dboxes, boxes, ref, act_dtype):
    _chk(dboxes, "dboxes", torch.float32); _chk(boxes, "boxes", torch.float32)
    levels, R, _ = boxes.shape
    ref_rows = ref.shape[0]
    assert dboxes.shape == boxes.shape and ref.shape == (ref_rows, 2) and R % ref_rows == 0
    dt_ = torch.empty((levels, R, 4), dtype=act_dtype, device=boxes.device)
    dref = torch.zeros((ref_rows, 2), dtype=torch.float32, device=boxes.device)
    call("fod_box_finish_bwd", _DT[act_dtype], ptr(dboxes), ptr(boxes), ptr(ref), ptr(dt_), ptr(dref),
         levels, R, ref_rows, stream())
    return dt_, dref


def match_cost(logits, boxes, tgt_labels, tgt_boxes, tgt_offset, ld_n, w_class, w_bbox, w_giou,
               alpha=0.25, gamma=2.0):
    _chk(logits, "logits", torch.float32); _chk(boxes, "boxes", torch.float32)
    Lv, B, M, Cc = logits.shape
    assert boxes.shape == (Lv, B, M, 4) and tgt_offset.dtype == torch.int32 and tgt_offset.numel() == B + 1
    cost = torch.zeros((Lv, B, M, ld_n), dtype=torch.float32, device=logits.device)
    call("fod_match_cost", ptr(logits), ptr(boxes), ptr(tgt_labels), ptr(tgt_boxes), ptr(tgt_offset),
         ptr(cost), Lv, B, M, Cc, ld_n, w_class, w_bbox, w_giou, alpha, gamma, stream())
    return cost


def lap_solve_batch_host(cost_cpu, n_cols, threads=8):
    assert cost_cpu.device.type == "cpu" and cost_cpu.dtype == torch.float32 and cost_cpu.is_contiguous()
    P, M, ld = cost_cpu.shape
    nc = torch.tensor(n_cols, dtype=torch.int32)
    assert nc.numel() == P
    out = torch.empty((P, M), dtype=torch.int32)
    call("fod_lap_solve_batch_host", cost_cpu.data_ptr(), P, M, ld, nc.data_ptr(), out.data_ptr(), threads)
    return out


def _num_boxes_args(num_boxes):
    if isinstance(num_boxes, torch.Tensor):
        _chk(num_boxes, "num_boxes", torch.float32); assert num_boxes.numel() == 1
        return 1.0, num_boxes
    return float(num_boxes), None


def set_loss_fwd(logits, boxes, match, tgt_labels, tgt_boxes, tgt_offset, num_boxes, alpha):
    Lv, B, M, Cc = logits.shape
    _chk(match, "match", torch.int32); assert match.shape == (Lv, B, M)
    out = torch.empty((Lv, 5), dtype=torch.float32, device=logits.device)
    nb, nb_dev = _num_boxes_args(num_boxes)
    call("fod_set_loss_fwd", ptr(logits), ptr(boxes), ptr(match), ptr(tgt_labels), ptr(tgt_boxes),
         ptr(tgt_offset), ptr(out), Lv, B, M, Cc, nb, ptr(nb_dev), alpha, stream())
    return out


def set_loss_bwd(logits, boxes, match, tgt_labels, tgt_boxes, g, num_boxes, alpha):
    Lv, B, M, Cc = logits.shape
    _chk(g, "g", torch.float32); assert g.shape == (Lv, 3)
    dlogits, dboxes = torch.empty_like(logits), torch.empty_like(boxes)
    nb, nb_dev = _num_boxes_args(num_boxes)
    call("fod_set_loss_bwd", ptr(logits), ptr(boxes), ptr(match), ptr(tgt_labels), ptr(tgt_boxes), ptr(g),
         ptr(dlogits), ptr(dboxes), Lv, B, M, Cc, nb, ptr(nb_dev), alpha, stream())
    return dlogits, dboxes


def pack_targets_dev(anno_boxes, anno_classes, anno_active, H, W):
    _chk(anno_boxes, "anno_boxes", torch.float32); _chk(anno_classes, "anno_classes", torch.int64)
    _chk(anno_active, "anno_active", torch.int64)
    B, N = anno_classes.shape
    assert anno_boxes.shape == (B, N, 4) and anno_active.shape == (B, N)
    dev = anno_boxes.device
    labels = torch.empty((B * N,), dtype=torch.int64, device=dev)
    boxes = torch.empty((B * N, 4), dtype=torch.float32, device=dev)
    offset = torch.empty((B + 1,), dtype=torch.int32, device=dev)
    count = torch.empty((1,), dtype=torch.float32, device=dev)
    call("fod_pack_targets", ptr(anno_boxes), ptr(anno_classes), ptr(anno_active), B, N, 1 / W, 1 / H, ptr(labels),
         ptr(boxes), ptr(offset), ptr(count), stream())
    return {"labels": labels, "boxes": boxes, "offset": offset, "count": count, "ld": N, "device": True}

# ... 100 lines not shown
```

include/fod.h:

```cpp
#ifndef FOD_H_
#define FOD_H_

#include <stddef.h>
#include <stdint.h>

#ifdef __cplusplus
extern "C" {
#endif

typedef struct ihipStream_t* fod_stream_t;

enum { FOD_F32 = 0, FOD_BF16 = 1 };
enum { FOD_OK = 0, FOD_ERR_ARG = 1, FOD_ERR_LAUNCH = 2, FOD_ERR_RUNTIME = 3 };

size_t fod_last_error(char* buf, size_t cap);
int fod_abi_version(void);
#define FOD_ABI_VERSION 15

int fod_knob_set(const char* name, const char* value);
int fod_knob_get(const char* name, char* out, size_t out_bytes);

enum { FOD_ROUTE_NT_SMALL = 0,
       FOD_ROUTE_NT_128 = 1,
       FOD_ROUTE_NT_BIG = 2 };
typedef struct fod_nt_route {
  int kernel;
  int tile_n;
  int stages;
  int interleave;
  int ksplit;
  int wants_split_ws;
} fod_nt_route;
enum { FOD_ROUTE_TN_SMALL = 0,
       FOD_ROUTE_TN_128 = 1,
       FOD_ROUTE_TN_BIG = 2 };
typedef struct fod_tn_route {
  int kernel;
  int bi, bj;
  int nsplit;
  int m_per_split;
  int xcd_order;
  int uses_partials_ws;
} fod_tn_route;

typedef struct fod_epilogue {
  const float* scale;
  const float* shift;
  const void* residual;
  long ld_residual;
  int residual_row_mod;
  const void* relu_mask;
  long ld_mask;
  int relu;
  int out_f32;
  void* split_ws;
  void* split_tickets;
} fod_epilogue;
#define FOD_NT_SPLIT_WS_FLOATS (64 * 8 * 4096)
#define FOD_NT_SPLIT_TICKETS 64
#define FOD_TN_WS_BYTES ((size_t)64 << 20)
enum { FOD_WS_NT_SPLIT = 0, FOD_WS_NT_SPLIT_TICKETS = 1, FOD_WS_TN_PARTIALS = 2, FOD_WS_ATTN_SPLIT_PER_TILE = 3,
       FOD_WS_DET = 4, FOD_WS_TN_MULTI_DET = 5 };
size_t fod_workspace_bytes(int kind);
#define FOD_DET_WS_BYTES ((size_t)16 << 20)
#define FOD_TN_MULTI_DET_WS_BYTES ((size_t)128 << 20)
#define FOD_TN_DET_MAX_SPLITS 4

int fod_gemm_nt(int dtype, const void* A, long lda, int a_row_mod, const void* B, long ldb, void* C,
                long ldc, int M, int N, int K, const fod_epilogue* epi, fod_stream_t stream);

int fod_gemm_nt_route(int dtype, long lda, int a_row_mod, long ldb, long ldc, int M, int N, int K,
                      const fod_epilogue* epi, fod_nt_route* out);

int fod_gemm_tn_acc(int dtype, const void* G, long ldg, const void* X, long ldx, float* dW, long ldw,
                    int M, int N1, int K2, const float* row_scale, float* colsum, int accumulate,
                    void* ws ,
                    size_t ws_bytes, fod_stream_t stream);
int fod_gemm_tn_route(int dtype, int M, int N1, int K2, long ldg, long ldx, long ldw, int has_row_scale,
                      int has_colsum, int det, size_t ws_bytes, fod_tn_route* out);

int fod_gemm_nt_grouped(int dtype, const void* A, long lda, int a_seg_len, long a_seg_stride, const void* B,
                        long ldb, void* C, long ldc, int c_seg_cols, long c_seg_stride, int M, int N, int K,
                        const fod_epilogue* epi,
                        int res_nseg, long res_seg_stride, fod_stream_t stream);
int fod_gemm_nt_batched(int dtype, int batches, const void* A, long lda, long a_batch, const void* B, long ldb,
                        long b_batch, void* C, long ldc, long c_batch, int M, int N, int K, const fod_epilogue* epi,
                        long shift_batch, long residual_batch, long mask_batch, fod_stream_t stream);
int fod_gemm_tn_grouped(int dtype, const void* G, long ldg, int g_seg_cols, long g_seg_stride, const void* X,
                        long ldx, float* dW, long ldw, int M, int N1, int K2, float* colsum, int accumulate,
                        fod_stream_t stream);

typedef struct fod_tn_job {
  const void* G;
  const void* X;
  float* dW;
  float* colsum;
  long ldg, ldx, ldw;
  int M, N1, K2;
  int accumulate;
  int g_seg_cols;
  int chain;
  long g_seg_stride;
  int m_per_split, nsplit;
} fod_tn_job;
int fod_gemm_tn_multi(const fod_tn_job* jobs, const int* blk_job, const int* blk_tile, int nblocks, fod_stream_t stream);
int fod_gemm_tn_multi_long(const fod_tn_job* jobs, const int* blk_job, const int* blk_local, int nblocks,
                           fod_stream_t stream);
int fod_tn_plan_long(int M, int rows_hint, int* m_per_split, int* nsplit);
int fod_gemm_tn_acc_det(int dtype, const void* G, long ldg, const void* X, long ldx, float* dW, long ldw,
                        int M, int N1, int K2, const float* row_scale, float* colsum, int accumulate,
                        void* ws, size_t ws_bytes, fod_stream_t stream);
int fod_gemm_tn_multi_long_det(const fod_tn_job* jobs, const int* blk_job, const int* blk_local, int nblocks,
                               const long* part_off, int njobs, size_t part_floats, void* ws, size_t ws_bytes,
                               fod_stream_t stream);

int fod_colsum_acc(int dtype, const void* G, long ldg, int M, int N, int group_rows, float* out,
                   fod_stream_t stream);
int fod_colsum_acc_det(int dtype, const void* G, long ldg, int M, int N, int group_rows, float* out, void* ws,
                       size_t ws_bytes, fod_stream_t stream);

typedef struct fod_permute_job {
  const void* src;
  void* dst;
  const float* scale;
  int src_dtype, dst_dtype;
  int d0, d1, d2;
  int valid1, valid2, scale_axis;
  long s0, s1, s2;
  long t0, t1;
} fod_permute_job;
int fod_multi_permute3(const fod_permute_job* jobs, const int* blk_job, const int* blk_chunk, int nblocks,
                       fod_stream_t stream);
int fod_multi_permute_chunk(void);
int fod_multi_permute_tiles(int d0, int d1, int d2, long s0, long s1, long s2);

typedef struct fod_conv_geom {
  int Nimg, H, W, Cin;
  int Ho, Wo, Cout;
  int kh, kw, stride, pad;
} fod_conv_geom;

int fod_conv2d_fwd(int dtype, const void* x, const void* w, void* y, const fod_conv_geom* g,
                   const fod_epilogue* epi, fod_stream_t stream);
int fod_conv_stem_fwd(int dtype, const void* xp, const void* w, void* y, int Nimg, int Hp, int Wp, int Ho, int Wo,
                      int Cout, const fod_epilogue* epi, fod_stream_t stream);
int fod_stem_pool_fwd(int dtype, const void* xp, const void* w, const float* shift, void* y, int Nimg, int Hp, int Wp,
                      int Ho, int Wo, int Cout, fod_stream_t stream);
int fod_conv2d_dgrad(int dtype, const void* dy, const void* w_t, void* dx, const fod_conv_geom* g,
                     const fod_epilogue* epi, fod_stream_t stream);
int fod_conv2d_wgrad_acc(int dtype, const void* dy, const void* x, float* dw, const fod_conv_geom* g,
                         const float* row_scale, int accumulate, void* ws ,
                         size_t ws_bytes, fod_stream_t stream);
int fod_conv2d_wgrad_acc_det(int dtype, const void* dy, const void* x, float* dw, const fod_conv_geom* g,
                             const float* row_scale, int accumulate, void* ws, size_t ws_bytes, fod_stream_t stream);
enum { FOD_CONV_FWD = 0, FOD_CONV_DGRAD = 1, FOD_CONV_WGRAD = 2 };
int fod_conv2d_route(int which, int dtype, const fod_conv_geom* g, const fod_epilogue* epi, int det, size_t ws_bytes,
                     void* out);

int fod_bottleneck_fused_fwd(int dtype, const void* x, const void* w1, const float* b1, const void* w2,
                             const float* b2, const void* w3, const float* b3, const void* wd, const float* bd,
                             void* out, int Nimg, int H, int W, int Cin, int mid, int Cout, fod_stream_t stream);

int fod_maxpool3x3s2(int dtype, const void* x, void* y, int Nimg, int H, int W, int C, int Ho, int Wo,
                     fod_stream_t stream);

int fod_nchw_to_nhwc(int dtype, const float* src, void* dst, int F, int C, int H, int W, int Cp, int inner,
                     long stride_outer, long stride_inner, fod_stream_t stream);

int fod_u8_nchw_to_nhwc(int dtype, const unsigned char* src, void* dst, int F, int C, int H, int W, int Cp,
                        int inner, long stride_outer, long stride_inner, const float* mean, const float* std,
// ... 193 lines not shown
```

include/fod_ext.h:

```cpp
#ifndef FOD_EXT_H_
#define FOD_EXT_H_

#include "fod.h"

#ifdef __cplusplus
extern "C" {
#endif

int fod_multi_ema(const long* pairs, const long* numel, const int* blk_tensor, const int* blk_chunk, int nblocks,
                  const long long* updates_dev, float decay, int warmup, fod_stream_t stream);
int fod_multi_swap(const long* pairs, const long* numel, const int* blk_tensor, const int* blk_chunk, int nblocks,
                   fod_stream_t stream);
int fod_multi_accum(const long* pairs, const long* numel, const int* blk_tensor, const int* blk_chunk, int nblocks,
                    int mode, float scale, fod_stream_t stream);
int fod_clip_crop_resize_photo(const unsigned char* src, float* dst, int B, int L, int C, int H0, int W0, int H, int W,
                               long src_stride_b, long src_stride_l, const int* plans, const float* mean,
                               const float* std, const float* photo, fod_stream_t stream);
int fod_render_boxes(const void* src, int src_is_u8, unsigned char* dst, int B, int L, int H, int W, long src_stride_b,
                     long src_stride_l, const int* frame_idx, const float* mean, const float* std, const float* boxes,
                     const int* labels, int N, const unsigned char* palette, int P, int thickness, fod_stream_t stream);
int fod_attn_maps(int dtype, int njobs, const void* const* ptrs, const int* query_idx, int Q, float* out,
                  const fod_attn_shape* shape, fod_stream_t stream);
int fod_render_attention(const void* src, int src_is_u8, unsigned char* dst, int B, int L, int J, int H, int W,
                         long src_stride_b, long src_stride_l, const int* frame_idx, const float* mean, const float* std,
                         const float* maps, int h, int w, long map_stride_b, long map_stride_j,
                         const float* colour_scale, const unsigned char* lut, float gain, float max_alpha,
                         fod_stream_t stream);
int fod_render_labels(unsigned char* pictures, int B, int H, int W, const float* boxes, const int* labels, int N,
                      const int* idents, const float* scores, const unsigned char* names, int n_names, int name_stride,
                      const unsigned char* palette, int P, const unsigned char* font, int font_first, int G, int FW,
                      int FH, int scale, int thickness, fod_stream_t stream);

#ifdef __cplusplus
}
#endif
#endif
```

Baseline: 109.1 frame-sequences/s.

## Fuse back-to-back LayerNorm pair with residual adds into single fwd/bwd kernels

```diff
diff --git a/future-object-detection_amd/csrc/api.cpp b/future-object-detection_amd/csrc/api.cpp
--- a/future-object-detection_amd/csrc/api.cpp
+++ b/future-object-detection_amd/csrc/api.cpp
@@ -70,6 +70,7 @@
     {"FOD_ATTN_PF", &Knobs::attn_pf, nullptr},
     {"FOD_FP8_STAGE", &Knobs::fp8_stage, nullptr},
     {"FOD_LN_BWD_GROUPS", &Knobs::ln_bwd_groups, nullptr},
+    {"FOD_LN_PAIR", &Knobs::ln_pair, nullptr},
     {"FOD_BNK_VERSION", &Knobs::bnk_version, nullptr},
 };
 
diff --git a/future-object-detection_amd/csrc/elementwise.hip b/future-object-detection_amd/csrc/elementwise.hip
--- a/future-object-detection_amd/csrc/elementwise.hip
+++ b/future-object-detection_amd/csrc/elementwise.hip
@@ -1,6 +1,7 @@
 #include <stdlib.h>
 
 #include "common.h"
+#include "../../include/fod_ext.h"
 #include "det_reduce.h"
 #include "knobs.h"
 
@@ -39,6 +40,47 @@
 #pragma unroll
   for (int i = 0; i < EPL; ++i) t[i] = from_f32<T>(v[i]);
   __builtin_memcpy(__builtin_assume_aligned(p, SliceAlign<T, EPL>::VALUE), t, EPL * sizeof(T));
+}
+
+template <int D, int EPL, int LPR>
+FOD_DEVINL void ln_row_stats(const float* v, float eps, float& mu, float& rs) {
+#pragma clang fp contract(off)
+  float s = 0.f;
+#pragma unroll
+  for (int i = 0; i < EPL; ++i) s += v[i];
+  mu = row_sum<LPR>(s) * (1.f / D);
+  float q = 0.f;
+#pragma unroll
+  for (int i = 0; i < EPL; ++i) {
+    const float d = v[i] - mu;
+    q = __builtin_fmaf(d, d, q);
+  }
+  rs = rsqrtf(__builtin_fmaf(row_sum<LPR>(q), 1.f / D, eps));
+}
+template <int EPL>
+FOD_DEVINL void ln_row_out(float* o, const float* v, float mu, float rs, const float* ga, const float* be) {
+#pragma clang fp contract(off)
+#pragma unroll
+  for (int i = 0; i < EPL; ++i) o[i] = __builtin_fmaf((v[i] - mu) * rs, ga[i], be[i]);
+}
+template <int D, int EPL, int LPR>
+FOD_DEVINL void ln_row_bwd(float* o, const float* d, float* xh, float mu, float rs, const float* ga, float* ag, float* ab) {
+#pragma clang fp contract(off)
+  float g[EPL];
+  float s1 = 0.f, s2 = 0.f;
+#pragma unroll
+  for (int i = 0; i < EPL; ++i) {
+    xh[i] = (xh[i] - mu) * rs;
+    g[i] = d[i] * ga[i];
+    s1 += g[i];
+    s2 = __builtin_fmaf(g[i], xh[i], s2);
+    ag[i] = __builtin_fmaf(d[i], xh[i], ag[i]);
+    ab[i] += d[i];
+  }
+  s1 = row_sum<LPR>(s1) * (1.f / D);
+  s2 = row_sum<LPR>(s2) * (1.f / D);
+#pragma unroll
+  for (int i = 0; i < EPL; ++i) o[i] = rs * __builtin_fmaf(-xh[i], s2, g[i] - s1);
 }
 
 template <typename T, int D, int LPR>
@@ -83,17 +125,22 @@
       }
       if (live) __builtin_memcpy(__builtin_assume_aligned(sum_out + r * D + c0, SliceAlign<T, EPL>::VALUE), st, EPL * sizeof(T));
     }
-    float s = 0.f;
-#pragma unroll
-    for (int i = 0; i < EPL; ++i) s += v[i];
-    const float mu = row_sum<LPR>(s) * (1.f / D);
-    float q = 0.f;
-#pragma unroll
-    for (int i = 0; i < EPL; ++i) q += (v[i] - mu) * (v[i] - mu);
-    const float rs = rsqrtf(row_sum<LPR>(q) * (1.f / D) + eps);
-    float o[EPL];
-#pragma unroll
-    for (int i = 0; i < EPL; ++i) o[i] = (v[i] - mu) * rs * ga[i] + be[i];
+    float mu, rs, o[EPL];
+    if constexpr (sizeof(T) == 4) {
+      float s = 0.f;
+#pragma unroll
+      for (int i = 0; i < EPL; ++i) s += v[i];
+      mu = row_sum<LPR>(s) * (1.f / D);
+      float q = 0.f;
+#pragma unroll
+      for (int i = 0; i < EPL; ++i) q += (v[i] - mu) * (v[i] - mu);
+      rs = rsqrtf(row_sum<LPR>(q) * (1.f / D) + eps);
+#pragma unroll
+      for (int i = 0; i < EPL; ++i) o[i] = (v[i] - mu) * rs * ga[i] + be[i];
+    } else {
+      ln_row_stats<D, EPL, LPR>(v, eps, mu, rs);
+      ln_row_out<EPL>(o, v, mu, rs, ga, be);
+    }
     if (live) {
       ln_store<T, EPL>(y + r * D + c0, o);
       if (sub == 0) {
@@ -131,28 +178,43 @@
     float d[EPL], g[EPL], xh[EPL];
     ln_load<T, EPL>(d, dy + row * D + c0);
     ln_load<T, EPL>(xh, xs + row * D + c0);
-    float s1 = 0.f, s2 = 0.f;
-#pragma unroll
-    for (int i = 0; i < EPL; ++i) {
-      xh[i] = (xh[i] - mu) * rs;
-      g[i] = d[i] * ga[i];
-      s1 += g[i];
-      s2 += g[i] * xh[i];
-    }
-    s1 = row_sum<LPR>(s1) * (1.f / D);
-    s2 = row_sum<LPR>(s2) * (1.f / D);
-    float o[EPL];
-#pragma unroll
-    for (int i = 0; i < EPL; ++i) o[i] = rs * (g[i] - s1 - xh[i] * s2);
-    ln_store<T, EPL>(dx + row * D + c0, o);
-#pragma unroll
-    for (int i = 0; i < EPL; ++i) {
-      if (DET) {
-        dgamma[row * (2 * D) + c0 + i] = d[i] * xh[i];
-        dgamma[row * (2 * D) + D + c0 + i] = d[i];
-      } else {
-        atomicAdd(dgamma + goff + i, d[i] * xh[i]);
-        atomicAdd(dbeta + goff + i, d[i]);
+    if constexpr (sizeof(T) == 4) {
+      float s1 = 0.f, s2 = 0.f;
+#pragma unroll
+      for (int i = 0; i < EPL; ++i) {
+        xh[i] = (xh[i] - mu) * rs;
+        g[i] = d[i] * ga[i];
+        s1 += g[i];
+        s2 += g[i] * xh[i];
+      }
+      s1 = row_sum<LPR>(s1) * (1.f / D);
+      s2 = row_sum<LPR>(s2) * (1.f / D);
+      float o[EPL];
+#pragma unroll
+      for (int i = 0; i < EPL; ++i) o[i] = rs * (g[i] - s1 - xh[i] * s2);
+      ln_store<T, EPL>(dx + row * D + c0, o);
+#pragma unroll
+      for (int i = 0; i < EPL; ++i) {
+        if (DET) {
+          dgamma[row * (2 * D) + c0 + i] = d[i] * xh[i];
+          dgamma[row * (2 * D) + D + c0 + i] = d[i];
+        } else {
+          atomicAdd(dgamma + goff + i, d[i] * xh[i]);
+          atomicAdd(dbeta + goff + i, d[i]);
+        }
+      }
+    } else {
+      ln_row_bwd<D, EPL, LPR>(g, d, xh, mu, rs, ga, ag, ab);
+      ln_store<T, EPL>(dx + row * D + c0, g);
+#pragma unroll
+      for (int i = 0; i < EPL; ++i) {
+        if (DET) {
+          dgamma[row * (2 * D) + c0 + i] = ag[i];
+          dgamma[row * (2 * D) + D + c0 + i] = ab[i];
+        } else {
+          atomicAdd(dgamma + goff + i, ag[i]);
+          atomicAdd(dbeta + goff + i, ab[i]);
+        }
       }
     }
     return;
@@ -162,25 +224,33 @@
     const bool live = row < rows;
     const long r = live ? row : rows - 1;
     const float mu = mean[r], rs = rstd[r];
-    float d[EPL], g[EPL], xh[EPL];
+    float d[EPL], xh[EPL], o[EPL];
     ln_load<T, EPL>(d, dy + r * D + c0);
     ln_load<T, EPL>(xh, xs + r * D + c0);
-    float s1 = 0.f, s2 = 0.f;
-#pragma unroll
-    for (int i = 0; i < EPL; ++i) {
-      if (!live) d[i] = 0.f;
-      xh[i] = (xh[i] - mu) * rs;
-      g[i] = d[i] * ga[i];
-      s1 += g[i];
-      s2 += g[i] * xh[i];
-      ag[i] += d[i] * xh[i];
-      ab[i] += d[i];
-    }
-    s1 = row_sum<LPR>(s1) * (1.f / D);
-    s2 = row_sum<LPR>(s2) * (1.f / D);
-    float o[EPL];
-#pragma unroll
-    for (int i = 0; i < EPL; ++i) o[i] = rs * (g[i] - s1 - xh[i] * s2);
+    if constexpr (sizeof(T) == 4) {
+      float g[EPL];
+      float s1 = 0.f, s2 = 0.f;
+#pragma unroll
+      for (int i = 0; i < EPL; ++i) {
+        if (!live) d[i] = 0.f;
+        xh[i] = (xh[i] - mu) * rs;
+        g[i] = d[i] * ga[i];
+        s1 += g[i];
+        s2 += g[i] * xh[i];
+        ag[i] += d[i] * xh[i];
+        ab[i] += d[i];
+      }
+      s1 = row_sum<LPR>(s1) * (1.f / D);
+      s2 = row_sum<LPR>(s2) * (1.f / D);
+#pragma unroll
+      for (int i = 0; i < EPL; ++i) o[i] = rs * (g[i] - s1 - xh[i] * s2);
+    } else {
+      if (!live) {
+#pragma unroll
+        for (int i = 0; i < EPL; ++i) d[i] = 0.f;
+      }
+      ln_row_bwd<D, EPL, LPR>(o, d, xh, mu, rs, ga, ag, ab);
+    }
     if (live) ln_store<T, EPL>(dx + r * D + c0, o);
   }
 #pragma unroll
@@ -206,6 +276,174 @@
     } else {
       atomicAdd(dgamma + c, sg[0][c] + sg[1][c] + sg[2][c] + sg[3][c]);
       atomicAdd(dbeta + c, sb[0][c] + sb[1][c] + sb[2][c] + sb[3][c]);
+    }
+  }
+}
+
+template <typename T, int D, int LPR>
+__global__ __launch_bounds__(256) void ln_fwd_pair_kernel(const T* __restrict__ x, const T* __restrict__ res2,
+                                                          T* __restrict__ sum2_out, const float* __restrict__ gamma_a,
+                                                          const float* __restrict__ beta_a, const T* __restrict__ e,
+                                                          int ediv, const float* __restrict__ gamma_b,
+                                                          const float* __restrict__ beta_b, const T* __restrict__ pos,
+                                                          int pmod, T* __restrict__ y3, T* __restrict__ xp,
+                                                          float* __restrict__ mean_a, float* __restrict__ rstd_a,
+                                                          float* __restrict__ mean_b, float* __restrict__ rstd_b,
+                                                          int rows, float eps) {
+  constexpr int EPL = D / LPR, RPW = 64 / LPR;
+  const int lane = threadIdx.x & 63;
+  const int sub = lane % LPR, rsel = lane / LPR;
+  const int c0 = sub * EPL;
+  const long rows_per_block = (long)(blockDim.x >> 6) * RPW;
+  for (long base = (long)blockIdx.x * rows_per_block + (threadIdx.x >> 6) * RPW; base < rows;
+       base += (long)gridDim.x * rows_per_block) {
+    const long row = base + rsel;
+    const bool live = row < rows;
+    const long r = live ? row : rows - 1;
+    float v[EPL], t[EPL], p[EPL];
+    ln_load<T, EPL>(v, x + r * D + c0);
+    ln_load<T, EPL>(t, e + res_row(r, ediv, 0) * D + c0);
+    if (xp) ln_load<T, EPL>(p, pos + res_row(r, 0, pmod) * D + c0);
+    if (res2) {
+      float u[EPL];
+      ln_load<T, EPL>(u, res2 + r * D + c0);
+      T st[EPL];
+#pragma unroll
+      for (int i = 0; i < EPL; ++i) {
+        v[i] += u[i];
+        st[i] = from_f32<T>(v[i]);
+        v[i] = to_f32(st[i]);
+      }
+      if (live) __builtin_memcpy(__builtin_assume_aligned(sum2_out + r * D + c0, SliceAlign<T, EPL>::VALUE), st, EPL * sizeof(T));
+    }
+    float w[EPL];
+    {
+      float ga[EPL], be[EPL];
+      __builtin_memcpy(ga, __builtin_assume_aligned(gamma_a + c0, SliceAlign<float, EPL>::VALUE), EPL * sizeof(float));
+      __builtin_memcpy(be, __builtin_assume_aligned(beta_a + c0, SliceAlign<float, EPL>::VALUE), EPL * sizeof(float));
+      float mu, rs;
+      ln_row_stats<D, EPL, LPR>(v, eps, mu, rs);
+      ln_row_out<EPL>(w, v, mu, rs, ga, be);
+#pragma unroll
+      for (int i = 0; i < EPL; ++i) w[i] = to_f32(from_f32<T>(to_f32(from_f32<T>(w[i])) + t[i]));
+      if (live && sub == 0) {
+        mean_a[r] = mu;
+        rstd_a[r] = rs;
+      }
+    }
+    {
+      float ga[EPL], be[EPL];
+      __builtin_memcpy(ga, __builtin_assume_aligned(gamma_b + c0, SliceAlign<float, EPL>::VALUE), EPL * sizeof(float));
+      __builtin_memcpy(be, __builtin_assume_aligned(beta_b + c0, SliceAlign<float, EPL>::VALUE), EPL * sizeof(float));
+      float mu, rs, o[EPL];
+      ln_row_stats<D, EPL, LPR>(w, eps, mu, rs);
+      ln_row_out<EPL>(o, w, mu, rs, ga, be);
+      T o3[EPL];
+#pragma unroll
+      for (int i = 0; i < EPL; ++i) o3[i] = from_f32<T>(o[i]);
+      if (live) {
+        __builtin_memcpy(__builtin_assume_aligned(y3 + r * D + c0, SliceAlign<T, EPL>::VALUE), o3, EPL * sizeof(T));
+        if (xp) {
+          float a[EPL];
+#pragma unroll
+          for (int i = 0; i < EPL; ++i) a[i] = to_f32(o3[i]) + p[i];
+          ln_store<T, EPL>(xp + r * D + c0, a);
+        }
+        if (sub == 0) {
+          mean_b[r] = mu;
+          rstd_b[r] = rs;
+        }
+      }
+    }
+  }
+}
+
+template <typename T, int D, int LPR, bool DET = false>
+__global__ __launch_bounds__(256) void ln_bwd_pair_kernel(const T* __restrict__ dy, const T* __restrict__ sum2,
+                                                          const float* __restrict__ mean_a,
+                                                          const float* __restrict__ rstd_a,
+                                                          const float* __restrict__ mean_b,
+                                                          const float* __restrict__ rstd_b,
+                                                          const float* __restrict__ gamma_a,
+                                                          const float* __restrict__ beta_a,
+                                                          const float* __restrict__ gamma_b, const T* __restrict__ e,
+                                                          int ediv, T* __restrict__ dsum3, T* __restrict__ dsum2,
+                                                          float* __restrict__ dgamma_a, float* __restrict__ dbeta_a,
+                                                          float* __restrict__ dgamma_b, float* __restrict__ dbeta_b,
+                                                          int rows) {
+  constexpr int EPL = D / LPR, RPW = 64 / LPR;
+  __shared__ float sg[2][4][D];
+  __shared__ float sb[2][4][D];
+  const int lane = threadIdx.x & 63, w = threadIdx.x >> 6;
+  const int sub = lane % LPR, rsel = lane / LPR;
+  const int c0 = sub * EPL;
+  float ga[EPL], ba[EPL], gb[EPL];
+  __builtin_memcpy(ga, __builtin_assume_aligned(gamma_a + c0, SliceAlign<float, EPL>::VALUE), EPL * sizeof(float));
+  __builtin_memcpy(ba, __builtin_assume_aligned(beta_a + c0, SliceAlign<float, EPL>::VALUE), EPL * sizeof(float));
+  __builtin_memcpy(gb, __builtin_assume_aligned(gamma_b + c0, SliceAlign<float, EPL>::VALUE), EPL * sizeof(float));
+  float aga[EPL], aba[EPL], agb[EPL], abb[EPL];
+#pragma unroll
+  for (int i = 0; i < EPL; ++i) aga[i] = aba[i] = agb[i] = abb[i] = 0.f;
+  for (long base = (long)blockIdx.x * (4 * RPW) + w * RPW; base < rows; base += (long)gridDim.x * (4 * RPW)) {
+    const long row = base + rsel;
+    const bool live = row < rows;
+    const long r = live ? row : rows - 1;
+    const float mua = mean_a[r], rsa = rstd_a[r], mub = mean_b[r], rsb = rstd_b[r];
+    float d[EPL], xa[EPL], xb[EPL], o[EPL];
+    ln_load<T, EPL>(d, dy + r * D + c0);
+    ln_load<T, EPL>(xa, sum2 + r * D + c0);
+    ln_load<T, EPL>(xb, e + res_row(r, ediv, 0) * D + c0);
+    ln_row_out<EPL>(o, xa, mua, rsa, ga, ba);
+#pragma unroll
+    for (int i = 0; i < EPL; ++i) {
+      if (!live) d[i] = 0.f;
+      xb[i] = to_f32(from_f32<T>(to_f32(from_f32<T>(o[i])) + xb[i]));
+    }
+    ln_row_bwd<D, EPL, LPR>(o, d, xb, mub, rsb, gb, agb, abb);
+    T st[EPL];
+#pragma unroll
+    for (int i = 0; i < EPL; ++i) {
+      st[i] = from_f32<T>(o[i]);
+      d[i] = live ? to_f32(st[i]) : 0.f;
+    }
+    if (live) __builtin_memcpy(__builtin_assume_aligned(dsum3 + r * D + c0, SliceAlign<T, EPL>::VALUE), st, EPL * sizeof(T));
+    ln_row_bwd<D, EPL, LPR>(o, d, xa, mua, rsa, ga, aga, aba);
+    if (live) ln_store<T, EPL>(dsum2 + r * D + c0, o);
+  }
+#pragma unroll
+  for (int i = 0; i < EPL; ++i) {
+#pragma unroll
+    for (int o = LPR; o < 64; o <<= 1) {
+      aga[i] += __shfl_xor(aga[i], o);
+      aba[i] += __shfl_xor(aba[i], o);
+      agb[i] += __shfl_xor(agb[i], o);
+      abb[i] += __shfl_xor(abb[i], o);
+    }
+  }
+  if (rsel == 0) {
+#pragma unroll
+    for (int i = 0; i < EPL; ++i) {
+      sg[0][w][c0 + i] = aga[i];
+      sb[0][w][c0 + i] = aba[i];
+      sg[1][w][c0 + i] = agb[i];
+      sb[1][w][c0 + i] = abb[i];
+    }
+  }
+  __syncthreads();
+  for (int c = threadIdx.x; c < D; c += 256) {
+#pragma unroll
+    for (int k = 0; k < 2; ++k) {
+      float* dg = k ? dgamma_b : dgamma_a;
+      float* db = k ? dbeta_b : dbeta_a;
+      const float tg = sg[k][0][c] + sg[k][1][c] + sg[k][2][c] + sg[k][3][c];
+      const float tb = sb[k][0][c] + sb[k][1][c] + sb[k][2][c] + sb[k][3][c];
+      if (DET) {
+        dg[(long)blockIdx.x * (2 * D) + c] = tg;
+        dg[(long)blockIdx.x * (2 * D) + D + c] = tb;
+      } else {
+        atomicAdd(dg + c, tg);
+        atomicAdd(db + c, tb);
+      }
     }
   }
 }
@@ -885,6 +1123,114 @@
   return det_reduce_launch(r, groups, stream);
 }
 
+static int ln_pair_check(const char* who, int dtype, int D, int rows, int res_row_div, int pos_row_mod) {
+  FOD_REQUIRE(dtype == FOD_BF16 && D == 256, "%s: unsupported (dtype %d, D = %d): bf16 rows of 256 only", who, dtype, D);
+  FOD_REQUIRE(rows > 0 && res_row_div >= 0 && pos_row_mod >= 0, "%s: bad args (%d rows, row div %d, row mod %d)", who,
+              rows, res_row_div, pos_row_mod);
+  return FOD_OK;
+}
+
+extern "C" int fod_layernorm_pair_fwd(int dtype, const void* x, const void* res2, void* sum2_out, const float* gamma_a,
+                                      const float* beta_a, const void* e, int res_row_div, const float* gamma_b,
+                                      const float* beta_b, const void* pos, int pos_row_mod, void* y3, void* xp,
+                                      float* mean_a, float* rstd_a, float* mean_b, float* rstd_b, int rows, int D,
+                                      float eps, hipStream_t stream) {
+  if (int rc = ln_pair_check("layernorm_pair_fwd", dtype, D, rows, res_row_div, pos_row_mod)) return rc;
+  FOD_REQUIRE(x && gamma_a && beta_a && e && gamma_b && beta_b && y3 && mean_a && rstd_a && mean_b && rstd_b,
+              "layernorm_pair_fwd: bad args");
+  FOD_REQUIRE((res2 != nullptr) == (sum2_out != nullptr), "layernorm_pair_fwd: res2 and sum2_out come together");
+  FOD_REQUIRE((pos != nullptr) == (xp != nullptr), "layernorm_pair_fwd: pos and xp come together");
+  FOD_REQUIRE((((uintptr_t)x | (uintptr_t)res2 | (uintptr_t)sum2_out | (uintptr_t)gamma_a | (uintptr_t)beta_a |
+                (uintptr_t)e | (uintptr_t)gamma_b | (uintptr_t)beta_b | (uintptr_t)pos | (uintptr_t)y3 | (uintptr_t)xp) % 16) == 0,
+              "layernorm_pair_fwd: operands must be 16-byte aligned");
+  using T = __bf16;
+  if (rows < 8192) {
+    hipLaunchKernelGGL((ln_fwd_pair_kernel<T, 256, 64>), dim3(grid_for(rows, 4)), dim3(256), 0, stream, (const T*)x,
+                       (const T*)res2, (T*)sum2_out, gamma_a, beta_a, (const T*)e, res_row_div, gamma_b, beta_b,
+                       (const T*)pos, pos_row_mod, (T*)y3, (T*)xp, mean_a, rstd_a, mean_b, rstd_b, rows, eps);
+  } else {
+    hipLaunchKernelGGL((ln_fwd_pair_kernel<T, 256, 16>), dim3(grid_for(rows, 16)), dim3(256), 0, stream, (const T*)x,
+                       (const T*)res2, (T*)sum2_out, gamma_a, beta_a, (const T*)e, res_row_div, gamma_b, beta_b,
+                       (const T*)pos, pos_row_mod, (T*)y3, (T*)xp, mean_a, rstd_a, mean_b, rstd_b, rows, eps);
+  }
+  FOD_LAUNCH_CHECK();
+  return FOD_OK;
+}
+
+static int ln_pair_bwd_grid(int rows) {
+  int grid = rows < 8192 ? grid_for(rows, 16) : grid_for(rows, 16 * ln_bwd_groups());
+  return grid > 512 ? 512 : grid;
+}
+
+static int ln_pair_bwd_check(const char* who, int dtype, const void* dy, const void* sum2, const float* mean_a,
+                             const float* rstd_a, const float* mean_b, const float* rstd_b, const float* gamma_a,
+                             const float* beta_a, const float* gamma_b, const void* e, int res_row_div, void* dsum3,
+                             void* dsum2, float* dgamma_a, float* dbeta_a, float* dgamma_b, float* dbeta_b, int rows,
+                             int D) {
+  if (int rc = ln_pair_check(who, dtype, D, rows, res_row_div, 0)) return rc;
+  FOD_REQUIRE(dy && sum2 && mean_a && rstd_a && mean_b && rstd_b && gamma_a && beta_a && gamma_b && e && dsum3 && dsum2 &&
+              dgamma_a && dbeta_a && dgamma_b && dbeta_b, "%s: bad args", who);
+  FOD_REQUIRE((((uintptr_t)dy | (uintptr_t)sum2 | (uintptr_t)gamma_a | (uintptr_t)beta_a | (uintptr_t)gamma_b |
+                (uintptr_t)e | (uintptr_t)dsum3 | (uintptr_t)dsum2) % 16) == 0, "%s: operands must be 16-byte aligned", who);
+  return FOD_OK;
+}
+
+#define LN_PAIR_BWD(DET, DGA, DBA, DGB, DBB)                                                                     \
+  do {                                                                                                           \
+    using T = __bf16;                                                                                            \
+    if (rows < 8192) {                                                                                           \
+      hipLaunchKernelGGL((ln_bwd_pair_kernel<T, 256, 64, DET>), dim3(grid), dim3(256), 0, stream, (const T*)dy,  \
+                         (const T*)sum2, mean_a, rstd_a, mean_b, rstd_b, gamma_a, beta_a, gamma_b, (const T*)e,  \
+                         res_row_div, (T*)dsum3, (T*)dsum2, DGA, DBA, DGB, DBB, rows);                           \
+    } else {                                                                                                     \
+      hipLaunchKernelGGL((ln_bwd_pair_kernel<T, 256, 16, DET>), dim3(grid), dim3(256), 0, stream, (const T*)dy,  \
+                         (const T*)sum2, mean_a, rstd_a, mean_b, rstd_b, gamma_a, beta_a, gamma_b, (const T*)e,  \
+                         res_row_div, (T*)dsum3, (T*)dsum2, DGA, DBA, DGB, DBB, rows);                           \
+    }                                                                                                            \
+  } while (0)
+
+extern "C" int fod_layernorm_pair_bwd(int dtype, const void* dy, const void* sum2, const float* mean_a,
+                                      const float* rstd_a, const float* mean_b, const float* rstd_b,
+                                      const float* gamma_a, const float* beta_a, const float* gamma_b, const void* e,
+                                      int res_row_div, void* dsum3, void* dsum2, float* dgamma_a, float* dbeta_a,
+                                      float* dgamma_b, float* dbeta_b, int rows, int D, hipStream_t stream) {
+  if (int rc = ln_pair_bwd_check("layernorm_pair_bwd", dtype, dy, sum2, mean_a, rstd_a, mean_b, rstd_b, gamma_a, beta_a,
+                                 gamma_b, e, res_row_div, dsum3, dsum2, dgamma_a, dbeta_a, dgamma_b, dbeta_b, rows, D))
+    return rc;
+  const int grid = ln_pair_bwd_grid(rows);
+  LN_PAIR_BWD(false, dgamma_a, dbeta_a, dgamma_b, dbeta_b);
+  FOD_LAUNCH_CHECK();
+  return FOD_OK;
+}
+
+extern "C" int fod_layernorm_pair_bwd_det(int dtype, const void* dy, const void* sum2, const float* mean_a,
+                                          const float* rstd_a, const float* mean_b, const float* rstd_b,
+                                          const float* gamma_a, const float* beta_a, const float* gamma_b,
+                                          const void* e, int res_row_div, void* dsum3, void* dsum2, float* dgamma_a,
+                                          float* dbeta_a, float* dgamma_b, float* dbeta_b, int rows, int D, void* ws,
+                                          size_t ws_bytes, hipStream_t stream) {
+  FOD_REQUIRE_SCRATCH("layernorm_pair_bwd_det", ws, ws_bytes, FOD_DET_WS_BYTES);
+  if (int rc = ln_pair_bwd_check("layernorm_pair_bwd_det", dtype, dy, sum2, mean_a, rstd_a, mean_b, rstd_b, gamma_a,
+                                 beta_a, gamma_b, e, res_row_div, dsum3, dsum2, dgamma_a, dbeta_a, dgamma_b, dbeta_b,
+                                 rows, D))
+    return rc;
+  const int grid = ln_pair_bwd_grid(rows);
+  float* part_a = reinterpret_cast<float*>(ws);
+  float* part_b = part_a + (long)grid * 2 * D;
+  LN_PAIR_BWD(true, part_a, nullptr, part_b, nullptr);
+  FOD_LAUNCH_CHECK();
+  for (int k = 0; k < 2; ++k) {
+    foddet::ReduceParams r{};
+    r.part = k ? part_b : part_a; r.part_stride = 2L * D; r.part_batch = (long)grid * 2 * D; r.part_total = r.part_batch; r.nparts = grid;
+    r.out0 = k ? dgamma_b : dgamma_a; r.n0 = D; r.cols0 = D; r.ld0 = D; r.out0_batch = D;
+    r.out1 = k ? dbeta_b : dbeta_a; r.n1 = D; r.out1_batch = D;
+    r.accumulate = 1;
+    if (int rc = det_reduce_launch(r, 1, stream)) return rc;
+  }
+  return FOD_OK;
+}
+#undef LN_PAIR_BWD
+
 struct ColsumJob {
   const void* g;
   void* out;
diff --git a/future-object-detection_amd/csrc/knobs.h b/future-object-detection_amd/csrc/knobs.h
--- a/future-object-detection_amd/csrc/knobs.h
+++ b/future-object-detection_amd/csrc/knobs.h
@@ -24,6 +24,7 @@
   int attn_pf = 1;
   int fp8_stage = 1;
   int ln_bwd_groups = 4;
+  int ln_pair = 1;
   int bnk_version = 4;
 };
 
diff --git a/future-object-detection_amd/future_od/models/transformer.py b/future-object-detection_amd/future_od/models/transformer.py
--- a/future-object-detection_amd/future_od/models/transformer.py
+++ b/future-object-detection_amd/future_od/models/transformer.py
@@ -374,12 +374,15 @@
         self.D, self.H = Dsrc, num_heads
         self.droprate = droprate
 
-    def forward(self, src, pos, other=None, attn_mask=None, key_padding_mask=None):
+    def pair_fits(self, src, pos):
+        return _fused_tail(self.mlp[3], self.droprate, self.training) and Fn.layer_norm_pair_fits(src, pos)
+
+    def forward(self, src, pos, other=None, attn_mask=None, key_padding_mask=None, xp=None, pair=None):
         _no_masks(attn_mask, key_padding_mask)
         D = self.D
         N = pos.shape[-2]
         add_pos = (lambda t: Fn.add(t, pos, b_row_mod=N)) if pos.dim() == 2 else (lambda t: Fn.add(t, pos))
-        fused = Fn.in_proj_self(src, pos, self.attn.in_proj_weight, self.attn.in_proj_bias) if other is None else None
+        fused = Fn.in_proj_self(src, pos, self.attn.in_proj_weight, self.attn.in_proj_bias, xp=xp) if other is None else None
         if fused is not None:
             src, q, k, v = fused
         elif other is None:
@@ -393,6 +396,12 @@
         fuse = _fused_tail(self.mlp[3], p, t)
         src, h = Fn.linear_keep(src, self.mlp[0].weight, self.mlp[0].bias, relu=True, grad_masked=fuse)
         h = Fn.dropout(h, p, t)
+        if pair is not None:
+            norm, e, queue, slot, want_xp = pair
+            assert fuse
+            o = Fn.linear(h, self.mlp[3].weight, self.mlp[3].bias, x_relu=True).view(src.shape)
+            return Fn.layer_norm_pair(src, o, e, N, self.norm2.weight, self.norm2.bias, norm.weight, norm.bias,
+                                      pos=pos if want_xp else None, res_queue=queue, res_slot=slot)
         return _add_norm(src, _Proj(h, self.mlp[3], a_relu=fuse), self.norm2, p, t)
 
 
@@ -411,8 +420,24 @@
             self.egodeep_attend = None
 
     def forward(self, x, pos, egodeep: Optional[Tensor] = None, prevout: Optional[Tensor] = None, memory=None,
-                imu_pre: Optional[Tensor] = None, imu_queue=None):
-        x = self.self_attn(x, pos)
+                imu_pre: Optional[Tensor] = None, imu_queue=None, xp: Optional[Tensor] = None, want_xp=None):
+        one_key = (egodeep is not None and self.egodeep_attend is not None and egodeep.dim() == 2
+                   and not self.egodeep_attend.per_token_masks())
+        alone = not (prevout is not None and self.prevout_attn is not None) \
+            and not (memory is not None and len(memory) > 0 and len(self.previmage_attn) > 0)
+        if one_key and alone and self.self_attn.pair_fits(x, pos):
+            e = imu_pre if imu_pre is not None else self.egodeep_attend.forward_single_key(egodeep)
+            e = Fn.dropout(e, self.egodeep_attend.droprate, self.training)
+            queue, slot = imu_queue if (imu_queue is not None and e is imu_pre) else (None, 0)
+            x, nxt = self.self_attn(x, pos, xp=xp, pair=(self.norm_eda, e, queue, slot, bool(want_xp)))
+            if torch.is_grad_enabled():
+                x = Fn.ZeroGradAnchor.apply(x, *self.egodeep_attend.dead_parameters())
+            return x if want_xp is None else (x, nxt)
+        x = self._forward_separate(x, pos, egodeep, prevout, memory, imu_pre, imu_queue, xp)
+        return x if want_xp is None else (x, None)
+
+    def _forward_separate(self, x, pos, egodeep, prevout, memory, imu_pre, imu_queue, xp):
+        x = self.self_attn(x, pos, xp=xp)
         if prevout is not None and self.prevout_attn is not None:
             x = self.prevout_attn(x, pos, other=prevout)
         if memory is not None:
@@ -451,10 +476,12 @@
                 and not any(b.training and b.droprate > 0.0 for b in blocks) and Fn.imu_branch_fits(egodeep, blocks)):
             queue = Fn.ResGradQueue(len(blocks)) if (SW.FOD_RES_GRAD_QUEUE and torch.is_grad_enabled()) else None
             pre = Fn.imu_branch(egodeep, blocks, queue=queue)
+        xp = None
         for i, layer in enumerate(self.layers):
+            want_xp = i + 1 < len(self.layers)
             if pre is not None:
-                x = layer(x, pos, egodeep, prevout, memory, imu_pre=pre[i],
-                          imu_queue=None if queue is None else (queue, i))
+                x, xp = layer(x, pos, egodeep, prevout, memory, imu_pre=pre[i],
+                              imu_queue=None if queue is None else (queue, i), xp=xp, want_xp=want_xp)
             else:
-                x = layer(x, pos, egodeep, prevout, memory)
+                x, xp = layer(x, pos, egodeep, prevout, memory, xp=xp, want_xp=want_xp)
         return x
diff --git a/future-object-detection_amd/future_od/native/functional.py b/future-object-detection_amd/future_od/native/functional.py
--- a/future-object-detection_amd/future_od/native/functional.py
+++ b/future-object-detection_amd/future_od/native/functional.py
@@ -6,6 +6,7 @@
 from .arena import ARENA, _ZeroArena, zeros_f32
 from .prepared import (CAT, PREP, STACK, _Job, _Prepared, _VEC, _pad_to, _wkey, prep_conv, prep_linear,
                        prep_stem)
+from .norm_pair import LayerNormPairFn, layer_norm_pair, layer_norm_pair_fits
 from .wgrad import WGRADS, _WgradQueue
 from ..switches import SW
 
@@ -70,13 +71,13 @@
 class LinearFn(Function):
 
     @staticmethod
-    def forward(ctx, x, weight, bias, relu, out_f32):
+    def forward(ctx, x, weight, bias, relu, out_f32, x_relu=False):
         dtype = x.dtype
         w = prep_linear(weight, dtype, False)
         N = weight.shape[0]
         y = ops.gemm_nt(x, w[:N] if w.shape[0] != N else w, shift=bias, relu=relu, out_f32=out_f32)
         y = y.view(*x.shape[:-1], N)
-        ctx.relu, ctx.out_f32 = relu, out_f32
+        ctx.relu, ctx.out_f32, ctx.x_relu = relu, out_f32, bool(x_relu)
         ctx.weight, ctx.bias = weight, bias
         ctx.has_bias = bias is not None
         ctx.save_for_backward(x, y if relu else None)
@@ -100,15 +101,18 @@
             g = ops.eltwise(L.EW_RELU_MASK, g, y.view(-1, N))
         dx = None
         if ctx.needs_input_grad[0]:
-            dx = ops.gemm_nt(g, prep_linear(weight, dtype, True)).view(x.shape)
+            dx = ops.gemm_nt(g, prep_linear(weight, dtype, True),
+                             relu_mask=x.view(-1, K) if ctx.x_relu else None).view(x.shape)
+        else:
+            assert not ctx.x_relu
         dw, db = _param_grads(weight, ctx.bias, g, x.view(-1, K), ctx.needs_input_grad[1], ctx.needs_input_grad[2], True)
         if Np != N:
             dw, db = (None if dw is None else dw[:N]), (None if db is None else db[:N])
-        return dx, dw, db, None, None
-
-
-def linear(x, weight, bias=None, relu=False, out_f32=False):
-    return LinearFn.apply(x.contiguous(), weight, bias, relu, out_f32)
+        return dx, dw, db, None, None, None
+
+
+def linear(x, weight, bias=None, relu=False, out_f32=False, x_relu=False):
+    return LinearFn.apply(x.contiguous(), weight, bias, relu, out_f32, x_relu)
 
 
 class LinearKeepFn(Function):
@@ -675,22 +679,25 @@
 class InProjSelfFn(Function):
 
     @staticmethod
-    def forward(ctx, src, pos, w, b, row_mod):
-        xp = ops.eltwise(L.EW_ADD, src, pos, b_row_mod=row_mod)
+    def forward(ctx, src, pos, w, b, row_mod, xp=None):
+        if xp is None:
+            xp = ops.eltwise(L.EW_ADD, src, pos, b_row_mod=row_mod)
         return (src.view_as(src),) + _in_proj_forward(ctx, xp, src, w, b)
 
     @staticmethod
     def backward(ctx, dkeep, dq, dk, dv):
         need = ctx.needs_input_grad[0]
         _, dsrc, dw, db = _in_proj_backward(ctx, dq, dk, dv, need, need, chained=True, dkeep=dkeep)
-        return dsrc, None, dw, db, None
-
-
-def in_proj_self(src, pos, weight, bias):
+        return dsrc, None, dw, db, None, None
+
+
+def in_proj_self(src, pos, weight, bias, xp=None):
     if pos.requires_grad or not SW.FOD_LINEAR_KEEP:
         return None
     row_mod = pos.shape[-2] if pos.dim() == 2 else 0
-    return InProjSelfFn.apply(src.contiguous(), pos.contiguous(), weight, bias, row_mod)
+    assert xp is None or (not xp.requires_grad and xp.shape == src.shape)
+    return InProjSelfFn.apply(src.contiguous(), pos.contiguous(), weight, bias, row_mod,
+                              None if xp is None else xp.contiguous())
 
 
 class InProjCrossFn(Function):
diff --git a/future-object-detection_amd/future_od/native/norm_pair.py b/future-object-detection_amd/future_od/native/norm_pair.py
--- /dev/null
+++ b/future-object-detection_amd/future_od/native/norm_pair.py
@@ -0,0 +1,53 @@
+import torch
+from torch.autograd import Function
+
+from . import ops
+from .arena import zeros_f32
+
+
+class LayerNormPairFn(Function):
+
+    @staticmethod
+    def forward(ctx, x, o, e, gamma_a, beta_a, gamma_b, beta_b, res_row_div, pos, pos_row_mod, res_queue=None, res_slot=0):
+        y3, xp, s, mean_a, rstd_a, mean_b, rstd_b = ops.layernorm_pair_fwd(
+            x, o, gamma_a, beta_a, e, res_row_div, gamma_b, beta_b, pos=pos, pos_row_mod=pos_row_mod)
+        ctx.save_for_backward(s, mean_a, rstd_a, mean_b, rstd_b, gamma_a, beta_a, gamma_b, e)
+        ctx.res_row_div, ctx.res_shape = res_row_div, e.shape
+        ctx.res_queue, ctx.res_slot = res_queue, res_slot
+        if xp is not None:
+            ctx.mark_non_differentiable(xp)
+        return y3, xp
+
+    @staticmethod
+    def backward(ctx, dy, _dxp=None):
+        s, mean_a, rstd_a, mean_b, rstd_b, gamma_a, beta_a, gamma_b, e = ctx.saved_tensors
+        D = gamma_a.numel()
+        dev = dy.device
+        dga, dba, dgb, dbb = (zeros_f32((D,), dev) for _ in range(4))
+        dsum3, dsum2 = ops.layernorm_pair_bwd(dy.contiguous(), s, mean_a, rstd_a, mean_b, rstd_b, gamma_a, beta_a, gamma_b, e,
+                                              ctx.res_row_div, dga, dba, dgb, dbb)
+        de = None
+        if ctx.needs_input_grad[2]:
+            rows, div = dsum3.numel() // D, ctx.res_row_div
+            if div and ctx.res_queue is not None and rows % div == 0:
+                de = ctx.res_queue.push(ctx.res_slot, dsum3.view(rows, D), rows // div, div, D).view(ctx.res_shape)
+            elif div:
+                out = zeros_f32(((rows - 1) // div + 1, D), dev)
+                ops.colsum_acc(dsum3.view(rows, D), out, group_rows=div)
+                de = ops.permute3_cast(out, dsum3.dtype, (1, out.shape[0], D), (0, D, 1), valid2=D).view(ctx.res_shape)
+            else:
+                de = dsum3.view(ctx.res_shape)
+        return (dsum2 if ctx.needs_input_grad[0] else None, dsum2 if ctx.needs_input_grad[1] else None, de, dga, dba, dgb, dbb,
+                None, None, None, None, None)
+
+
+def layer_norm_pair_fits(x, pos=None):
+    return ops.layernorm_pair_fits(x, x.shape[-1]) and (pos is None or not pos.requires_grad)
+
+
+def layer_norm_pair(x, o, e, res_row_div, gamma_a, beta_a, gamma_b, beta_b, pos=None, res_queue=None, res_slot=0):
+    assert pos is None or not pos.requires_grad
+    row_mod = pos.shape[-2] if pos is not None and pos.dim() == 2 else 0
+    return LayerNormPairFn.apply(x.contiguous(), None if o is None else o.contiguous(), e.contiguous(), gamma_a, beta_a,
+                                 gamma_b, beta_b, res_row_div, None if pos is None else pos.contiguous(), row_mod,
+                                 res_queue, res_slot)
diff --git a/future-object-detection_amd/future_od/native/ops.py b/future-object-detection_amd/future_od/native/ops.py
--- a/future-object-detection_amd/future_od/native/ops.py
+++ b/future-object-detection_amd/future_od/native/ops.py
@@ -1024,6 +1024,53 @@
     return dx
 
 
+def layernorm_pair_fits(x, D):
+    return x.dtype == torch.bfloat16 and D == 256 and x.is_cuda and L.knob("FOD_LN_PAIR") != "0"
+
+
+def layernorm_pair_fwd(x, res2, gamma_a, beta_a, e, res_row_div, gamma_b, beta_b, pos=None, pos_row_mod=0, eps=1e-5):
+    _chk(x, "x"); _chk(e, "e", x.dtype)
+    D = x.shape[-1]
+    rows = x.numel() // D
+    for t in (gamma_a, beta_a, gamma_b, beta_b):
+        _chk(t, "gamma/beta", torch.float32); assert t.numel() == D
+    assert e.shape[-1] == D and e.numel() // D >= ((rows - 1) // res_row_div + 1 if res_row_div else rows)
+    s = x
+    if res2 is not None:
+        _chk(res2, "res2", x.dtype); assert res2.numel() == x.numel()
+        s = torch.empty_like(x)
+    xp = None
+    if pos is not None:
+        _chk(pos, "pos", x.dtype)
+        assert pos.shape[-1] == D and pos.numel() // D >= (min(pos_row_mod, rows) if pos_row_mod else rows)
+        xp = torch.empty_like(x)
+    y3 = torch.empty_like(x)
+    stats = [torch.empty(rows, dtype=torch.float32, device=x.device) for _ in range(4)]
+    call("fod_layernorm_pair_fwd", dt(x), ptr(x), ptr(res2), ptr(s) if res2 is not None else None, ptr(gamma_a), ptr(beta_a),
+         ptr(e), res_row_div, ptr(gamma_b), ptr(beta_b), ptr(pos), pos_row_mod, ptr(y3), ptr(xp), *(ptr(t) for t in stats),
+         rows, D, eps, stream(), tag="fod_layernorm_fwd")
+    return (y3, xp, s, *stats)
+
+
+def layernorm_pair_bwd(dy, sum2, mean_a, rstd_a, mean_b, rstd_b, gamma_a, beta_a, gamma_b, e, res_row_div, dgamma_a, dbeta_a,
+                       dgamma_b, dbeta_b):
+    _chk(dy, "dy"); _chk(sum2, "sum2", dy.dtype); _chk(e, "e", dy.dtype)
+    D = dy.shape[-1]
+    rows = dy.numel() // D
+    assert sum2.numel() == dy.numel() and all(t.numel() == rows for t in (mean_a, rstd_a, mean_b, rstd_b))
+    for t in (gamma_a, beta_a, gamma_b, dgamma_a, dbeta_a, dgamma_b, dbeta_b):
+        _chk(t, "gamma/beta/dgamma/dbeta", torch.float32); assert t.numel() == D
+    dsum3, dsum2 = torch.empty_like(dy), torch.empty_like(dy)
+    args = (dt(dy), ptr(dy), ptr(sum2), ptr(mean_a), ptr(rstd_a), ptr(mean_b), ptr(rstd_b), ptr(gamma_a), ptr(beta_a),
+            ptr(gamma_b), ptr(e), res_row_div, ptr(dsum3), ptr(dsum2), ptr(dgamma_a), ptr(dbeta_a), ptr(dgamma_b),
+            ptr(dbeta_b), rows, D)
+    if SW.FOD_DETERMINISTIC:
+        call("fod_layernorm_pair_bwd_det", *args, *det_workspace(dy.device), stream(), tag="fod_layernorm_bwd")
+    else:
+        call("fod_layernorm_pair_bwd", *args, stream(), tag="fod_layernorm_bwd")
+    return dsum3, dsum2
+
+
 def eltwise(op, a, b=None, c=None, b_row_div=0, b_row_mod=0, alpha=1.0, out=None):
     _chk(a, "a")
     cols = a.shape[-1]
diff --git a/include/fod.h b/include/fod.h
--- a/include/fod.h
+++ b/include/fod.h
@@ -15,7 +15,7 @@
 
 size_t fod_last_error(char* buf, size_t cap);
 int fod_abi_version(void);
-#define FOD_ABI_VERSION 15
+#define FOD_ABI_VERSION 16
 
 int fod_knob_set(const char* name, const char* value);
 int fod_knob_get(const char* name, char* out, size_t out_bytes);
diff --git a/include/fod_ext.h b/include/fod_ext.h
--- a/include/fod_ext.h
+++ b/include/fod_ext.h
@@ -30,6 +30,21 @@
                       const int* idents, const float* scores, const unsigned char* names, int n_names, int name_stride,
                       const unsigned char* palette, int P, const unsigned char* font, int font_first, int G, int FW,
                       int FH, int scale, int thickness, fod_stream_t stream);
+int fod_layernorm_pair_fwd(int dtype, const void* x, const void* res2, void* sum2_out, const float* gamma_a,
+                           const float* beta_a, const void* e, int res_row_div, const float* gamma_b,
+                           const float* beta_b, const void* pos, int pos_row_mod, void* y3, void* xp, float* mean_a,
+                           float* rstd_a, float* mean_b, float* rstd_b, int rows, int D, float eps,
+                           fod_stream_t stream);
+int fod_layernorm_pair_bwd(int dtype, const void* dy, const void* sum2, const float* mean_a, const float* rstd_a,
+                           const float* mean_b, const float* rstd_b, const float* gamma_a, const float* beta_a,
+                           const float* gamma_b, const void* e, int res_row_div, void* dsum3, void* dsum2,
+                           float* dgamma_a, float* dbeta_a, float* dgamma_b, float* dbeta_b, int rows, int D,
+                           fod_stream_t stream);
+int fod_layernorm_pair_bwd_det(int dtype, const void* dy, const void* sum2, const float* mean_a, const float* rstd_a,
+                               const float* mean_b, const float* rstd_b, const float* gamma_a, const float* beta_a,
+                               const float* gamma_b, const void* e, int res_row_div, void* dsum3, void* dsum2,
+                               float* dgamma_a, float* dbeta_a, float* dgamma_b, float* dbeta_b, int rows, int D,
+                               void* ws, size_t ws_bytes, fod_stream_t stream);
 
 #ifdef __cplusplus
 }
```

After: 109.5 frame-sequences/s, median of 6. Within noise of the previous version (+0.3%).
